# wei-zeng98/piano-a2s

Measured on AMD Instinct MI355X. Metric: training clips/sec (12 s, 5-bar), higher is better.
Workload: dtype f32

## Files before the change

### include/a2s.h

```cpp
#ifndef A2S_H
#define A2S_H
#include <stddef.h>
#include <stdint.h>
#ifdef __cplusplus
extern "C" {
#endif

#define A2S_OK 0
#define A2S_ERR_ARG (-1)
#define A2S_ERR_HIP (-2)
#define A2S_ERR_WORKSPACE (-3)

const char* a2s_last_error(void);
int a2s_version(void);
long long a2s_launch_count(void);

int a2s_gemm_f32(void* stream, int M, int N, int K, float alpha, const float* A, long sAm, long sAk,
                 const float* B, long sBk, long sBn, float beta, float* C, long ldc, const float* bias, int act,
                 int batch, long bsA, long bsB, long bsC, int splitk, float* workspace, size_t workspace_bytes);
int a2s_gemm_f32_affine(void* stream, int M, int N, int K, float alpha, const float* A, long sAm, long sAk, const float* B, long sBk,
                        long sBn, float beta, float* C, long ldc, const float* bias, int act, int batch, long bsA, long bsB, long bsC,
                        int splitk, float* workspace, size_t workspace_bytes, const float* a_scale, const float* a_shift, int a_period,
                        const float* b_scale, const float* b_shift, int b_period);
int a2s_gemm_f32_bnstats(void* stream, int M, int N, int K, const float* A, long sAm, long sAk, const float* B, long sBk, long sBn, float* C, long ldc,
                         const float* y, const float* mean, const float* invstd, const float* scale, const float* shift, int period, float* partial);
int a2s_gemm_f32_affine_scaled(void* stream, int M, int N, int K, float alpha, const float* A, long sAm, long sAk, const float* B, long sBk,
                               long sBn, float beta, float* C, long ldc, const float* bias, int act, int batch, long bsA, long bsB, long bsC,
                               int splitk, float* workspace, size_t workspace_bytes, const float* a_scale, const float* a_shift, int a_period,
                               const float* b_scale, const float* b_shift, int b_period, const float* a_absmax, const float* b_absmax);
int a2s_gemm_f32_bnstats_scaled(void* stream, int M, int N, int K, const float* A, long sAm, long sAk, const float* B, long sBk, long sBn, float* C, long ldc,
                                const float* y, const float* mean, const float* invstd, const float* scale, const float* shift, int period, float* partial,
                                const float* a_absmax, const float* b_absmax);
int a2s_linear_dgrad_bnstats(void* stream, int M, int N, int K, const float* dz, long lda, const float* Wt, float* da, long ldc, const float* y,
                             const float* mean, const float* invstd, const float* scale, const float* shift, int period, float* partial,
                             const float* dz_absmax, const float* w_absmax, float* workspace, size_t workspace_bytes, float* da_absmax_out);
int a2s_linear_fwd(void* stream, int M, int N, int K, const float* y, long lda, const float* W, float* z, long ldc, const float* scale, const float* shift,
                   int period, const float* y_absmax, const float* w_absmax, float* workspace, size_t workspace_bytes);
int a2s_linear_fwd_eligible(int M, int N, int K, int period);
int a2s_linear_wgrad(void* stream, int M, int N, int K, const float* dz, long ldz, const float* y, long lda, float* G, long ldg, const float* scale,
                     const float* shift, int period, const float* dz_absmax, const float* y_absmax, float* workspace, size_t workspace_bytes);
size_t a2s_linear_wgrad_ws_bytes(int M, int K);
int a2s_linear_wgrad_eligible(int M, int N, int K, int period);
int a2s_tallk_wgrad(void* stream, int M, int Np, int K, const float* P, long ldp, const float* A, long lda, float* G, long ldg, int transposed, float* bias,
                    const float* p_absmax, const float* a_absmax, float* workspace, size_t workspace_bytes);
size_t a2s_tallk_wgrad_ws_bytes(int M, int Np, int K);
int a2s_tallk_wgrad_eligible(int M, int Np, int K, long ldp, long lda, long ldg, int transposed);
size_t a2s_linear_dgrad_ws_bytes(int N, int K);
int a2s_linear_dgrad_blocks(int M);
int a2s_linear_dgrad_eligible(int M, int N, int K, int period);
int a2s_absmax(void* stream, const float* x, long n, float* out);
int a2s_gemm_bnstats_blocks(int M, int period);
size_t a2s_gemm_workspace_bytes(int M, int N, int batch, int splitk);
int a2s_gemm_pick_splitk(int M, int N, int K, int batch);
void a2s_gemm_debug_tile(int cfg);
int a2s_debug_set(const char* key, int value);
int a2s_debug_get(const char* key);
int a2s_env_check(void);
int a2s_persist_abort_latch(void* device_word);

int a2s_conv3x3(void* stream, const float* x, const float* w, float* y, const float* in_scale, const float* in_shift,
                float* stat_partial, int B, int T, int F, int Cin, int Cout, int flip, float* workspace);
int a2s_conv3x3_ranged(void* stream, const float* x, const float* w, float* y, const float* in_scale, const float* in_shift, const float* in_absmax,
                       float* stat_partial, float* out_absmax, int B, int T, int F, int Cin, int Cout, float* workspace);
int a2s_conv3x3_stat_blocks(int B, int T, int F, int Cin);
int a2s_conv3x3_dgrad_bnstats(void* stream, const float* dy, const float* w, float* g, const float* yl, const float* yl_mean, const float* yl_invstd,
                              const float* yl_scale, const float* yl_shift, float* stat_partial, int B, int T, int F, int Cin, int Cout,
                              float* workspace);
int a2s_bn_bwd_from_partial(void* stream, const float* g, const float* x, const float* mean, const float* invstd, const float* scale, const float* shift,
                            float* dgamma, float* dbeta, float* dx , const float* partial, int nblocks, float* c12, long rows, int C, int F);
int a2s_conv3x3_dgrad_bnstats_scaled(void* stream, const float* dy, const float* w, float* g, const float* yl, const float* yl_mean, const float* yl_invstd,
                                     const float* yl_scale, const float* yl_shift, float* stat_partial, int B, int T, int F, int Cin, int Cout,
                                     float* workspace, const float* dy_absmax);
int a2s_conv3x3_dgrad_bnstats_ranged(void* stream, const float* dy, const float* w, float* g, const float* yl, const float* yl_mean, const float* yl_invstd,
                                     const float* yl_scale, const float* yl_shift, float* stat_partial, int B, int T, int F, int Cin, int Cout,
                                     float* workspace, const float* dy_absmax, float* g_absmax_out);
int a2s_bn_bwd_from_partial_amax(void* stream, const float* g, const float* x, const float* mean, const float* invstd, const float* scale, const float* shift,
                                 float* dgamma, float* dbeta, float* dx, const float* partial, int nblocks, float* c12, long rows, int C, int F,
                                 float* dx_absmax);
size_t a2s_conv3x3_workspace_floats(int Cin);
int a2s_bn_finalize(void* stream, const float* partial, int nblocks, int C, double count, const float* gamma,
                    const float* beta, float* running_mean, float* running_var, long long* num_batches_tracked,
                    float* mean, float* invstd, float* scale, float* shift, float eps, float momentum, int training);
int a2s_bn_relu_apply(void* stream, const float* x, float* y, const float* scale, const float* shift, long n, int C, int F);
int a2s_col_stats(void* stream, const float* x, float* partial, long rows, int C, int rows_per_block);
int a2s_bn1d_relu_dropout(void* stream, const float* x, float* y, const float* scale, const float* shift,
                          const uint8_t* keep_mask, float inv_keep, long n, int C);

int a2s_gru_gates_fwd(void* stream, const float* gi, long ldgi, const float* gh, long ldgh, const float* hprev, long ldhp,
                      float* hout, long ldho, float* hout2, long ldho2, float* save, int R, int H);
int a2s_gru_seq_fwd(void* stream, const float* gi_all, long gi_bstride, long gi_tstride, const float* w_hh,
                    const float* b_hh, float* out, long out_bstride, long out_tstride, float* hbuf, float* gh,
                    float* save, float* hn, int B, int T, int H, int reverse, float* workspace, size_t workspace_bytes);

int a2s_attn_step_fwd(void* stream, const float* keys, const float* enc, const float* q, long ldq, const float* v,
                      float* ctx, long ldctx, float* ctx2, long ldctx2, float* attw, int B, int T, int H,
                      const int* n_done, int n_rows_total, float* workspace);
int a2s_attn_step_fwd_rows(void* stream, const float* keys, const float* enc, const float* q, long ldq, const float* v, float* ctx,
                           long ldctx, float* ctx2, long ldctx2, float* attw, int R, int T, int H, float* workspace, int n_clips,
                           const int* clip_order, const int* clip_rank, const int* row_until, int n_active, int step);
size_t a2s_attn_workspace_floats(int B, int T, int H);
size_t a2s_attn_workspace_floats_fused(int n_clips, int T, int H, int groups);

int a2s_log_softmax_rows(void* stream, const float* x, long ldx, float* y, long ldy, int* argmax_out, int R, int V);
int a2s_embed_rows(void* stream, const float* table, const long long* ids64, const int* ids32, long id_stride,
                   int const_id, float* out, long ldo, int col0, int R, int E, const uint8_t* keep_mask, float inv_keep);

typedef struct a2s_note_dec_args {
    const float* attn_w; const float* attn_b; const float* attn_v;
    const float* w_ih; const float* w_hh; const float* b_ih; const float* b_hh;
    const float* out_w; const float* out_b; const float* emb;
    const float* keys; const float* enc;
    float* h; float* x; float* q; float* gates; float* attw; float* o;
    float* gh; float* gi; float* logits;
    float* probs; long probs_bstride;
    const long long* gt; long gt_bstride;
    const uint8_t* tf_flags;
    const uint8_t* drop; float inv_keep;
    int* argmax_out; long am_bstride;
    int* eos_seen; long long* lengths; int* n_done;
    int* steps_exec;
    float* attn_ws;
    float* gemm_ws; size_t gemm_ws_bytes;
    int* t_base;
    const int* clip_order;
    const int* clip_rank;
    const int* row_until;
    const int* n_active;
    int n_clips;
    const int* m_active;
    const int* row_list;
    const int* n_rows_active;
    int R, T, H, E, V, steps, poll, eos_id;
    int use_graph;
    float* step_ws; size_t step_ws_floats;
    const int* tf_flags_dev;
// ... 201 lines not shown
```

### piano_a2s_amd/csrc/a2s_api.hip

```cpp
#define A2S_SWITCHES_IMPL
#include "a2s_internal.h"

thread_local char a2s_err_msg[512] = {0};
long long a2s_launch_counter = 0;

#define ST ((hipStream_t)stream)

extern "C" {

const char* a2s_last_error(void) { return a2s_err_msg; }
int a2s_version(void) { return 1; }
long long a2s_launch_count(void) { return __atomic_load_n(&a2s_launch_counter, __ATOMIC_RELAXED); }

int a2s_gemm_f32(void* stream, int M, int N, int K, float alpha, const float* A, long sAm, long sAk, const float* B, long sBk,
                 long sBn, float beta, float* C, long ldc, const float* bias, int act, int batch, long bsA, long bsB, long bsC,
                 int splitk, float* workspace, size_t workspace_bytes) {
    return a2s_gemm_impl(ST, M, N, K, alpha, A, sAm, sAk, B, sBk, sBn, beta, C, ldc, bias, act, batch, bsA, bsB, bsC, splitk,
                         workspace, workspace_bytes);
}
int a2s_gemm_f32_affine(void* stream, int M, int N, int K, float alpha, const float* A, long sAm, long sAk, const float* B, long sBk,
                        long sBn, float beta, float* C, long ldc, const float* bias, int act, int batch, long bsA, long bsB, long bsC,
                        int splitk, float* workspace, size_t workspace_bytes, const float* a_scale, const float* a_shift, int a_period,
                        const float* b_scale, const float* b_shift, int b_period) {
    return a2s_gemm_affine_impl(ST, M, N, K, alpha, A, sAm, sAk, B, sBk, sBn, beta, C, ldc, bias, act, batch, bsA, bsB, bsC, splitk,
                                workspace, workspace_bytes, a_scale, a_shift, a_period, b_scale, b_shift, b_period,
                                nullptr, nullptr, nullptr, nullptr, nullptr, nullptr, 0, 0, nullptr, nullptr);
}
int a2s_gemm_f32_affine_scaled(void* stream, int M, int N, int K, float alpha, const float* A, long sAm, long sAk, const float* B, long sBk,
                               long sBn, float beta, float* C, long ldc, const float* bias, int act, int batch, long bsA, long bsB, long bsC,
                               int splitk, float* workspace, size_t workspace_bytes, const float* a_scale, const float* a_shift, int a_period,
                               const float* b_scale, const float* b_shift, int b_period, const float* a_absmax, const float* b_absmax) {
    return a2s_gemm_affine_impl(ST, M, N, K, alpha, A, sAm, sAk, B, sBk, sBn, beta, C, ldc, bias, act, batch, bsA, bsB, bsC, splitk,
                                workspace, workspace_bytes, a_scale, a_shift, a_period, b_scale, b_shift, b_period,
                                nullptr, nullptr, nullptr, nullptr, nullptr, nullptr, 0, 1, a_absmax, b_absmax);
}
int a2s_gemm_f32_bnstats_scaled(void* stream, int M, int N, int K, const float* A, long sAm, long sAk, const float* B, long sBk, long sBn, float* C, long ldc,
                                const float* y, const float* mean, const float* invstd, const float* scale, const float* shift, int period, float* partial,
                                const float* a_absmax, const float* b_absmax) {
    return a2s_gemm_affine_impl(ST, M, N, K, 1.f, A, sAm, sAk, B, sBk, sBn, 0.f, C, ldc, nullptr, 0, 1, 0, 0, 0, 1, nullptr, 0,
                                nullptr, nullptr, 0, nullptr, nullptr, 0, y, mean, invstd, scale, shift, partial, period, 1, a_absmax, b_absmax);
}
int a2s_absmax(void* stream, const float* x, long n, float* out) { return a2s_absmax_impl(ST, x, n, out); }
int a2s_linear_dgrad_bnstats(void* stream, int M, int N, int K, const float* dz, long lda, const float* Wt, float* da, long ldc, const float* y,
                             const float* mean, const float* invstd, const float* scale, const float* shift, int period, float* partial,
                             const float* dz_absmax, const float* w_absmax, float* workspace, size_t workspace_bytes, float* da_absmax_out) {
    return a2s_linear_dgrad_bnstats_impl(ST, M, N, K, dz, lda, Wt, 1, K, da, ldc, y, mean, invstd, scale, shift, period, partial, dz_absmax, w_absmax,
                                         workspace, workspace_bytes, da_absmax_out);
}
size_t a2s_linear_dgrad_ws_bytes(int N, int K) { return a2s_linear_dgrad_ws_bytes_impl(N, K); }
int a2s_linear_fwd(void* stream, int M, int N, int K, const float* y, long lda, const float* W, float* z, long ldc, const float* scale, const float* shift,
                   int period, const float* y_absmax, const float* w_absmax, float* workspace, size_t workspace_bytes) {
    return a2s_linear_fwd_impl(ST, M, N, K, y, lda, W, z, ldc, scale, shift, period, y_absmax, w_absmax, workspace, workspace_bytes);
}
int a2s_linear_wgrad(void* stream, int M, int N, int K, const float* dz, long ldz, const float* y, long lda, float* G, long ldg, const float* scale,
                     const float* shift, int period, const float* dz_absmax, const float* y_absmax, float* workspace, size_t workspace_bytes) {
    return a2s_linear_wgrad_impl(ST, M, N, K, dz, ldz, y, lda, G, ldg, scale, shift, period, dz_absmax, y_absmax, workspace, workspace_bytes);
}
size_t a2s_linear_wgrad_ws_bytes(int M, int K) { return a2s_linear_wgrad_ws_bytes_impl(M, K); }
int a2s_linear_wgrad_eligible(int M, int N, int K, int period) { return a2s_linear_wgrad_ok(M, N, K, 256, 4, 4, period, nullptr, nullptr, nullptr) ? 1 : 0; }
int a2s_tallk_wgrad(void* stream, int M, int Np, int K, const float* P, long ldp, const float* A, long lda, float* G, long ldg, int transposed, float* bias,
                    const float* p_absmax, const float* a_absmax, float* workspace, size_t workspace_bytes) {
    return a2s_tallk_wgrad_impl(ST, M, Np, K, P, ldp, A, lda, G, ldg, transposed, bias, p_absmax, a_absmax, workspace, workspace_bytes);
}
size_t a2s_tallk_wgrad_ws_bytes(int M, int Np, int K) { return a2s_tallk_wgrad_ws_bytes_impl(M, Np, K); }
int a2s_tallk_wgrad_eligible(int M, int Np, int K, long ldp, long lda, long ldg, int transposed) {
    return a2s_tallk_wgrad_ok(M, Np, K, ldp, lda, ldg, transposed, nullptr, nullptr, nullptr, nullptr) ? 1 : 0;
}
int a2s_linear_fwd_eligible(int M, int N, int K, int period) { return a2s_linear_fwd_ok(M, N, K, 4, 4, period, nullptr, nullptr, nullptr) ? 1 : 0; }
int a2s_linear_dgrad_blocks(int M) { return a2s_linear_dgrad_blocks_impl(M); }
int a2s_linear_dgrad_eligible(int M, int N, int K, int period) {
    return a2s_linear_dgrad_ok(M, N, K, 4, 1, K, 4, period, nullptr, nullptr, nullptr, nullptr) ? 1 : 0;
}
int a2s_gemm_f32_bnstats(void* stream, int M, int N, int K, const float* A, long sAm, long sAk, const float* B, long sBk, long sBn, float* C, long ldc,
                         const float* y, const float* mean, const float* invstd, const float* scale, const float* shift, int period, float* partial) {
    return a2s_gemm_affine_impl(ST, M, N, K, 1.f, A, sAm, sAk, B, sBk, sBn, 0.f, C, ldc, nullptr, 0, 1, 0, 0, 0, 1, nullptr, 0,
                                nullptr, nullptr, 0, nullptr, nullptr, 0, y, mean, invstd, scale, shift, partial, period, 0, nullptr, nullptr);
}
int a2s_gemm_bnstats_blocks(int M, int period) { return a2s_cdiv(M, 128) * a2s_gemm_bnstats_slots(period); }
size_t a2s_gemm_workspace_bytes(int M, int N, int batch, int splitk) { return a2s_gemm_workspace_bytes_impl(M, N, batch, splitk); }
int a2s_gemm_pick_splitk(int M, int N, int K, int batch) { return a2s_gemm_pick_splitk_impl(M, N, K, batch); }
void a2s_gemm_debug_tile(int cfg) { a2s_gemm_debug_tile_impl(cfg); }
size_t a2s_note_step_workspace_floats(int H, int E) { return a2s_note_step_workspace_floats_impl(H, E); }
int a2s_debug_set(const char* key, int value) {
    if (!key) return A2S_ERR_ARG;
    const int id = a2s_switch_find(key);
    if (id >= 0) { a2s_switch_store(id, value); return A2S_OK; }
    if (!strcmp(key, "attn_deferred_fast")) { a2s_attn_deferred_fast = value ? 1 : 0; return A2S_OK; }
    if (!strcmp(key, "tallk_wgrad")) { a2s_tallk_wgrad_on = value ? 1 : 0; return A2S_OK; }
    if (!strcmp(key, "tallk_wgrad_max_splits")) { a2s_tallk_wgrad_max_splits = value > 0 ? value : 0; return A2S_OK; }
    if (!strcmp(key, "gemm_tile")) { a2s_gemm_debug_tile_impl(value); return A2S_OK; }
    snprintf(a2s_err_msg, sizeof(a2s_err_msg), "a2s_debug_set: unknown key %s", key);
    return A2S_ERR_ARG;
}
int a2s_env_check(void) {
    if (const char* e = a2s_switch_env_error()) A2S_FAIL(A2S_ERR_ARG, "%s: expected a decimal number >= 0", e);
    return A2S_OK;
}

int a2s_persist_abort_latch(void* device_word) { a2s_persist_latch_set(device_word); return A2S_OK; }

int a2s_debug_get(const char* key) {
    if (!key) return -1;
    const int id = a2s_switch_find(key);
    if (id == A2S_SW_attn_pair_fused_rows) return a2s_attn_pair_fused_rows();
    if (id >= 0) return a2s_sw((a2s_switch)id);
    if (!strcmp(key, "attn_pair_launches")) return (int)a2s_attn_pair_launches();
    if (!strcmp(key, "attn_pair_bwd_launches")) return (int)a2s_attn_pair_bwd_launches();
    if (!strcmp(key, "attn_deferred_fast")) return a2s_attn_deferred_fast;
    if (!strcmp(key, "tallk_wgrad")) return a2s_tallk_wgrad_on;
    if (!strcmp(key, "tallk_wgrad_max_splits")) return a2s_tallk_wgrad_max_splits;
    if (!strcmp(key, "tallk_wgrad_launches")) return (int)a2s_tallk_wgrad_launches();
    if (!strcmp(key, "attn_dk_ahead_launches")) return (int)a2s_attn_dk_ahead_launches();
    if (!strcmp(key, "attn_denc_launches")) return (int)a2s_attn_denc_launches();
    if (!strcmp(key, "dec_mid_launches")) return a2s_dec_mid_launches();
    if (!strcmp(key, "dec_persist_launches")) return a2s_dec_persist_launches();
    if (!strcmp(key, "edit_distance_launches")) return (int)a2s_edit_distance_launches();
    if (!strcmp(key, "conv_rows16_c20_launches")) return (int)a2s_conv_rows16_c20_launches();
    if (!strcmp(key, "device_cus")) return a2s_device_geometry().cus;
    if (!strcmp(key, "device_xccs")) return a2s_device_geometry().xccs;
    return -1;
}

int a2s_conv3x3(void* stream, const float* x, const float* w, float* y, const float* in_scale, const float* in_shift,
                float* stat_partial, int B, int T, int F, int Cin, int Cout, int flip, float* workspace) {
    return a2s_conv3x3_impl(ST, x, w, y, in_scale, in_shift, stat_partial, B, T, F, Cin, Cout, flip, workspace, nullptr, nullptr, nullptr, nullptr, nullptr, nullptr,
                            nullptr, nullptr);
}
int a2s_conv3x3_ranged(void* stream, const float* x, const float* w, float* y, const float* in_scale, const float* in_shift, const float* in_absmax,
                       float* stat_partial, float* out_absmax, int B, int T, int F, int Cin, int Cout, float* workspace) {
    return a2s_conv3x3_impl(ST, x, w, y, in_scale, in_shift, stat_partial, B, T, F, Cin, Cout, 0, workspace, nullptr, nullptr, nullptr, nullptr, nullptr, nullptr,
                            in_absmax, out_absmax);
}
int a2s_conv3x3_dgrad_bnstats(void* stream, const float* dy, const float* w, float* g, const float* yl, const float* yl_mean, const float* yl_invstd,
                              const float* yl_scale, const float* yl_shift, float* stat_partial, int B, int T, int F, int Cin, int Cout,
                              float* workspace) {
    if (!yl) { snprintf(a2s_err_msg, sizeof(a2s_err_msg), "conv3x3_dgrad_bnstats: yl is required"); return A2S_ERR_ARG; }
    return a2s_conv3x3_impl(ST, dy, w, g, nullptr, nullptr, stat_partial, B, T, F, Cin, Cout, 1, workspace, yl, yl_mean, yl_invstd, yl_scale, yl_shift, nullptr, nullptr, nullptr);
}
int a2s_conv3x3_dgrad_bnstats_scaled(void* stream, const float* dy, const float* w, float* g, const float* yl, const float* yl_mean, const float* yl_invstd,
                                     const float* yl_scale, const float* yl_shift, float* stat_partial, int B, int T, int F, int Cin, int Cout,
                                     float* workspace, const float* dy_absmax) {
    if (!yl) { snprintf(a2s_err_msg, sizeof(a2s_err_msg), "conv3x3_dgrad_bnstats_scaled: yl is required"); return A2S_ERR_ARG; }
    return a2s_conv3x3_impl(ST, dy, w, g, nullptr, nullptr, stat_partial, B, T, F, Cin, Cout, 1, workspace, yl, yl_mean, yl_invstd, yl_scale, yl_shift, dy_absmax, nullptr, nullptr);
}
int a2s_conv3x3_dgrad_bnstats_ranged(void* stream, const float* dy, const float* w, float* g, const float* yl, const float* yl_mean, const float* yl_invstd,
                                     const float* yl_scale, const float* yl_shift, float* stat_partial, int B, int T, int F, int Cin, int Cout,
                                     float* workspace, const float* dy_absmax, float* g_absmax_out) {
    if (!yl) { snprintf(a2s_err_msg, sizeof(a2s_err_msg), "conv3x3_dgrad_bnstats_ranged: yl is required"); return A2S_ERR_ARG; }
    return a2s_conv3x3_impl(ST, dy, w, g, nullptr, nullptr, stat_partial, B, T, F, Cin, Cout, 1, workspace, yl, yl_mean, yl_invstd, yl_scale, yl_shift, dy_absmax, nullptr, g_absmax_out);
}
int a2s_bn_bwd_from_partial(void* stream, const float* g, const float* x, const float* mean, const float* invstd, const float* scale, const float* shift,
                            float* dgamma, float* dbeta, float* dx, const float* partial, int nblocks, float* c12, long rows, int C, int F) {
    return a2s_bn_bwd_from_partial_impl(ST, g, x, mean, invstd, scale, shift, dgamma, dbeta, dx, partial, nblocks, c12, rows, C, F, nullptr);
}
int a2s_bn_bwd_from_partial_amax(void* stream, const float* g, const float* x, const float* mean, const float* invstd, const float* scale, const float* shift,
                                 float* dgamma, float* dbeta, float* dx, const float* partial, int nblocks, float* c12, long rows, int C, int F,
                                 float* dx_absmax) {
    return a2s_bn_bwd_from_partial_impl(ST, g, x, mean, invstd, scale, shift, dgamma, dbeta, dx, partial, nblocks, c12, rows, C, F, dx_absmax);
}
size_t a2s_conv3x3_workspace_floats(int Cin) { return a2s_conv3x3_workspace_floats_impl(Cin); }
int a2s_conv3x3_stat_blocks(int B, int T, int F, int Cin) { return a2s_conv3x3_stat_blocks_impl(B, T, F, Cin); }
int a2s_bn_finalize(void* stream, const float* partial, int nblocks, int C, double count, const float* gamma, const float* beta,
                    float* running_mean, float* running_var, long long* nbt, float* mean, float* invstd, float* scale,
                    float* shift, float eps, float momentum, int training) {
    return a2s_bn_finalize_impl(ST, partial, nblocks, C, count, gamma, beta, running_mean, running_var, nbt, mean, invstd, scale,
                                shift, eps, momentum, training);
}
int a2s_bn_relu_apply(void* stream, const float* x, float* y, const float* scale, const float* shift, long n, int C, int F) {
    return a2s_bn_relu_apply_impl(ST, x, y, scale, shift, n, C, F);
}
int a2s_col_stats(void* stream, const float* x, float* partial, long rows, int C, int rows_per_block) {
    return a2s_col_stats_impl(ST, x, partial, rows, C, rows_per_block);
}
int a2s_bn1d_relu_dropout(void* stream, const float* x, float* y, const float* scale, const float* shift, const uint8_t* keep_mask,
                          float inv_keep, long n, int C) {
    return a2s_bn1d_relu_dropout_impl(ST, x, y, scale, shift, keep_mask, inv_keep, n, C);
}
int a2s_gru_gates_fwd(void* stream, const float* gi, long ldgi, const float* gh, long ldgh, const float* hprev, long ldhp,
                      float* hout, long ldho, float* hout2, long ldho2, float* save, int R, int H) {
    return a2s_gru_gates_fwd_impl(ST, gi, ldgi, gh, ldgh, hprev, ldhp, hout, ldho, hout2, ldho2, save, R, H);
}
int a2s_gru_seq_fwd(void* stream, const float* gi_all, long gi_bstride, long gi_tstride, const float* w_hh, const float* b_hh,
                    float* out, long out_bstride, long out_tstride, float* hbuf, float* gh, float* save, float* hn, int B, int T,
                    int H, int reverse, float* workspace, size_t workspace_bytes) {
    return a2s_gru_seq_fwd_impl(ST, gi_all, gi_bstride, gi_tstride, w_hh, b_hh, out, out_bstride, out_tstride, hbuf, gh, save, hn,
                                B, T, H, reverse, workspace, workspace_bytes);
}
int a2s_attn_step_fwd(void* stream, const float* keys, const float* enc, const float* q, long ldq, const float* v, float* ctx,
                      long ldctx, float* ctx2, long ldctx2, float* attw, int B, int T, int H, const int* n_done, int n_rows_total, float* workspace) {
    return a2s_attn_step_fwd_impl(ST, keys, enc, q, ldq, v, ctx, ldctx, ctx2, ldctx2, attw, B, T, H, n_done, n_rows_total, workspace, nullptr);
}
int a2s_attn_step_fwd_rows(void* stream, const float* keys, const float* enc, const float* q, long ldq, const float* v, float* ctx,
// ... 285 lines not shown
```

### piano_a2s_amd/csrc/a2s_common.h

```cpp
#pragma once
#include <hip/hip_runtime.h>
#include <stdint.h>
#include <stdio.h>
#include <string.h>

#define A2S_OK 0
#define A2S_ERR_ARG (-1)
#define A2S_ERR_HIP (-2)
#define A2S_ERR_WORKSPACE (-3)

extern thread_local char a2s_err_msg[512];

#define A2S_FAIL(code, ...)                                   \
    do {                                                      \
        snprintf(a2s_err_msg, sizeof(a2s_err_msg), __VA_ARGS__); \
        return (code);                                        \
    } while (0)

#define A2S_REQUIRE(cond, ...)                 \
    do {                                       \
        if (!(cond)) A2S_FAIL(A2S_ERR_ARG, __VA_ARGS__); \
    } while (0)

#define A2S_CHECK_LAUNCH(name)                                                        \
// ... 64 lines not shown
}
#define A2S_DPP_QUAD_1032 0xB1
#define A2S_DPP_QUAD_2301 0x4E
#define A2S_DPP_ROW_HALF_MIRROR 0x141
#define A2S_DPP_ROW_MIRROR 0x140
#define A2S_DPP_ROW_BCAST15 0x142
#define A2S_DPP_ROW_BCAST31 0x143
__device__ __forceinline__ float wave_sum_lane63(float v) {
    v += dpp_take<A2S_DPP_QUAD_1032>(0.f, v);
    v += dpp_take<A2S_DPP_QUAD_2301>(0.f, v);
    v += dpp_take<A2S_DPP_ROW_HALF_MIRROR>(0.f, v);
    v += dpp_take<A2S_DPP_ROW_MIRROR>(0.f, v);
    v += dpp_take<A2S_DPP_ROW_BCAST15, 0xA>(0.f, v);
    v += dpp_take<A2S_DPP_ROW_BCAST31, 0xC>(0.f, v);
    return v;
}
__device__ __forceinline__ float wave_sum(float v) {
    return __builtin_bit_cast(float, __builtin_amdgcn_readlane(__builtin_bit_cast(int, wave_sum_lane63(v)), 63));
}
__device__ __forceinline__ float wave_max(float v) {
    v = fmaxf(v, dpp_take<A2S_DPP_QUAD_1032>(v, v));
    v = fmaxf(v, dpp_take<A2S_DPP_QUAD_2301>(v, v));
    v = fmaxf(v, dpp_take<A2S_DPP_ROW_HALF_MIRROR>(v, v));
    v = fmaxf(v, dpp_take<A2S_DPP_ROW_MIRROR>(v, v));
    v = fmaxf(v, dpp_take<A2S_DPP_ROW_BCAST15, 0xA, false>(v, v));
    v = fmaxf(v, dpp_take<A2S_DPP_ROW_BCAST31, 0xC, false>(v, v));
    return __builtin_bit_cast(float, __builtin_amdgcn_readlane(__builtin_bit_cast(int, v), 63));
}
__device__ __forceinline__ float attn_merge_weight(float mg, float lg, bool have, float& m_out, float& inv_l_out) {
#pragma clang fp contract(off)
    const float m = wave_max(mg);
    const float d = mg - m;
    const float e = have ? __expf(d) : 0.f;
    const float t = lg * e;
    const float l = wave_sum(t);
    m_out = m;
    inv_l_out = 1.f / l;
    return e / l;
}
struct GruCellGrad { float dr, dz, dn, dnr, dhz; };
__device__ __forceinline__ GruCellGrad gru_cell_bwd(float dh, float rg, float zg, float ng, float ghn, float hp) {
#pragma clang fp contract(off)
    GruCellGrad o;
    o.dn = dh * (1.f - zg) * (1.f - ng * ng);
    o.dz = dh * (hp - ng) * zg * (1.f - zg);
    o.dr = o.dn * ghn * rg * (1.f - rg);
    o.dnr = o.dn * rg;
    o.dhz = dh * zg;
    return o;
}
__device__ __forceinline__ double wave_sum_d(double v) {
#pragma unroll
    for (int o = 32; o > 0; o >>= 1) v += __shfl_xor(v, o, 64);
    return v;
}

__device__ __forceinline__ float block_sum(float v, float* red) {
    v = wave_sum(v);
    const int w = threadIdx.x >> 6, nw = (blockDim.x + 63) >> 6;
    __syncthreads();
    if ((threadIdx.x & 63) == 0) red[w] = v;
    __syncthreads();
    float t = 0.f;
    for (int i = 0; i < nw; ++i) t += red[i];
    return t;
}
__device__ __forceinline__ float block_max(float v, float* red) {
    v = wave_max(v);
    const int w = threadIdx.x >> 6, nw = (blockDim.x + 63) >> 6;
    __syncthreads();
    if ((threadIdx.x & 63) == 0) red[w] = v;
    __syncthreads();
    float t = red[0];
    for (int i = 1; i < nw; ++i) t = fmaxf(t, red[i]);
    return t;
}

__device__ __forceinline__ float fast_tanh(float x) {
    x = fminf(fmaxf(x, -15.f), 15.f);
    const float e = __expf(2.f * x);
    return fmaf(-2.f, __builtin_amdgcn_rcpf(e + 1.f), 1.f);
}
__device__ __forceinline__ float exp2x_clamped(float x) { return __expf(2.f * fminf(fmaxf(x, -43.f), 43.f)); }
__device__ __forceinline__ float tanh_ek(float ek, float eq) { return fmaf(-2.f, __builtin_amdgcn_rcpf(fmaf(ek, eq, 1.f)), 1.f); }
__device__ __forceinline__ float sech2_ek(float ek, float eq) {
    const float r = __builtin_amdgcn_rcpf(fmaf(ek, eq, 1.f));
    return 4.f * r * (1.f - r);
}
__device__ __forceinline__ float fast_sigmoid(float x) {
    x = fminf(fmaxf(x, -30.f), 30.f);
    return __builtin_amdgcn_rcpf(1.f + __expf(-x));
}
typedef __attribute__((ext_vector_type(8))) __bf16 bf16x8;
typedef __attribute__((ext_vector_type(2))) __bf16 bf16x2;
typedef __attribute__((ext_vector_type(2))) float f32x2;
__device__ __forceinline__ void split3_pair(float x0, float x1, unsigned& p0, unsigned& p1, unsigned& p2) {
    f32x2 v = {x0, x1};
    p0 = __builtin_bit_cast(unsigned, __builtin_convertvector(v, bf16x2));
    v[0] -= __uint_as_float(p0 << 16); v[1] -= __uint_as_float(p0 & 0xffff0000u);
    p1 = __builtin_bit_cast(unsigned, __builtin_convertvector(v, bf16x2));
    v[0] -= __uint_as_float(p1 << 16); v[1] -= __uint_as_float(p1 & 0xffff0000u);
    p2 = __builtin_bit_cast(unsigned, __builtin_convertvector(v, bf16x2));
}

typedef __attribute__((ext_vector_type(8))) _Float16 f16x8;
typedef __attribute__((ext_vector_type(2))) _Float16 f16x2;
__device__ __forceinline__ void split2_pair_f16(float x0, float x1, unsigned& p0, unsigned& p1) {
    f32x2 v = {x0, x1};
    const f16x2 t0 = __builtin_convertvector(v, f16x2);
    p0 = __builtin_bit_cast(unsigned, t0);
    asm("v_fma_mix_f32 %0, %1, -1.0, %0 op_sel_hi:[1,0,0]" : "+v"(v[0]) : "v"(p0));
    asm("v_fma_mix_f32 %0, %1, -1.0, %0 op_sel:[1,0,0] op_sel_hi:[1,0,0]" : "+v"(v[1]) : "v"(p0));
    p1 = __builtin_bit_cast(unsigned, __builtin_convertvector(v, f16x2));
}
__device__ __forceinline__ void block_absmax_to(float* __restrict__ out, float am, float* red) {
    am = block_max(am, red);
    if (threadIdx.x == 0) {
        const unsigned bits = __float_as_uint(am);
        if (bits > __hip_atomic_load(reinterpret_cast<unsigned*>(out), __ATOMIC_RELAXED, __HIP_MEMORY_SCOPE_AGENT))
            atomicMax(reinterpret_cast<unsigned*>(out), bits);
    }
}
__device__ __forceinline__ int pow2_scale_exp(float amax, int target) {
    if (!(amax > 0.f) || !isfinite(amax)) return 0;
    const int k = target - ilogbf(amax);
    return min(max(k, -96), 96);
}

#endif
```

### piano_a2s_amd/csrc/a2s_gemm.hip

```cpp
#include "a2s_internal.h"

struct GemmArgs {
    const float* A; const float* B; float* C; const float* bias;
    int M, N, K;
    long sAm, sAk, sBk, sBn, ldc;
    float alpha, beta;
    int act;
    int batch; long bsA, bsB, bsC;
    int splitk; int kchunk;
    float* partial;
    int vecA, vecB;
    const float* a_scale; const float* a_shift; int a_period;
    const float* b_scale; const float* b_shift; int b_period;
    const float* ep_y; const float* ep_mean; const float* ep_invstd; const float* ep_scale; const float* ep_shift;
    float* ep_partial; int ep_period, ep_channels, ep_slots;
    int two_term; const float* a_absmax; const float* b_absmax;
};

#define GEMM_BK 32
#ifndef GEMM_DEPTH
#define GEMM_DEPTH 1
#endif

template <int ROWS, bool KC> struct LdsTile {
// ... 309 lines not shown
#pragma unroll
            for (int i = 0; i < TM; ++i)
#pragma unroll
                for (int j = 0; j < TN; ++j)
#pragma unroll
                    for (int r = 0; r < 4; ++r) acc[i][j][r] *= unscale;
        }
    } else {
        constexpr int D = (BM * BN <= 64 * 64) ? GEMM_DEPTH : 1;
        f32x4 qa[D][NLA], qb[D][NLB];
        float ga[D][NLA][2], gb[D][NLB][2];
#pragma unroll
        for (int i = 0; i < NLA; ++i) { qa[0][i] = ra[i]; ga[0][i][0] = fa[i][0]; ga[0][i][1] = fa[i][1]; }
#pragma unroll
        for (int i = 0; i < NLB; ++i) { qb[0][i] = rb[i]; gb[0][i][0] = fb[i][0]; gb[0][i][1] = fb[i][1]; }
#pragma unroll
        for (int d = 1; d < D; ++d) {
            if (d < ntiles) {
                const int k0 = kbeg + d * GEMM_BK;
                tile_load<BM, A_KC, NLA>(A, g.sAm, g.sAk, m0, k0, g.M, kend, g.vecA, qa[d], ga[d], g.a_scale, g.a_shift, g.a_period);
                tile_load<BN, B_KC, NLB>(B, g.sBn, g.sBk, n0, k0, g.N, kend, g.vecB, qb[d], gb[d], g.b_scale, g.b_shift, g.b_period);
            }
        }
        for (int t0 = 0; t0 < ntiles; t0 += D) {
#pragma unroll
            for (int d = 0; d < D; ++d) {
                const int t = t0 + d;
                if (t >= ntiles) break;
                float* la = lds + (t & 1) * (LA::SIZE + LB::SIZE);
                float* lb = la + LA::SIZE;
                tile_store<BM, A_KC, NLA>(la, qa[d], ga[d], m0, kbeg + t * GEMM_BK, g.M, kend, g.a_scale, g.a_shift, g.a_period);
                tile_store<BN, B_KC, NLB>(lb, qb[d], gb[d], n0, kbeg + t * GEMM_BK, g.N, kend, g.b_scale, g.b_shift, g.b_period);
                __syncthreads();
                if (t + D < ntiles) {
                    const int k0 = kbeg + (t + D) * GEMM_BK;
                    tile_load<BM, A_KC, NLA>(A, g.sAm, g.sAk, m0, k0, g.M, kend, g.vecA, qa[d], ga[d], g.a_scale, g.a_shift, g.a_period);
                    tile_load<BN, B_KC, NLB>(B, g.sBn, g.sBk, n0, k0, g.N, kend, g.vecB, qb[d], gb[d], g.b_scale, g.b_shift, g.b_period);
                }
#pragma unroll
                for (int ks = 0; ks < GEMM_BK / 4; ++ks) {
                    float a[TM], b[TN];
#pragma unroll
                    for (int i = 0; i < TM; ++i) a[i] = la[LA::at(wm + i * 16 + lr, ks * 4 + lk)];
#pragma unroll
                    for (int j = 0; j < TN; ++j) b[j] = lb[LB::at(wn + j * 16 + lr, ks * 4 + lk)];
#pragma unroll
                    for (int i = 0; i < TM; ++i)
#pragma unroll
                        for (int j = 0; j < TN; ++j)
                            acc[i][j] = __builtin_amdgcn_mfma_f32_16x16x4f32(b[j], a[i], acc[i][j], 0, 0, 0);
                }
            }
        }
    }


    const bool partial = g.splitk > 1;
    float* C = partial ? g.partial + (long)blockIdx.z * g.M * g.N : g.C + (long)zb * g.bsC;
    const long ldc = partial ? g.N : g.ldc;
    const bool vec_c = (ldc % 4 == 0) && (((uintptr_t)C & 15) == 0);
    const int ep_c0 = g.ep_y ? n0 / g.ep_period : 0;
    float ep_s[2][2] = {{0.f, 0.f}, {0.f, 0.f}};
#pragma unroll
    for (int i = 0; i < TM; ++i) {
        const int m = m0 + wm + i * 16 + lr;
        if (m >= g.M) continue;
#pragma unroll
        for (int j = 0; j < TN; ++j) {
            const int n = n0 + wn + j * 16 + lk * 4;
            if (n >= g.N) continue;
            f32x4 v = acc[i][j];
            float* dst = C + (long)m * ldc + n;
            const bool full = vec_c && n + 3 < g.N;
            if (!partial) {
                f32x4 old = {0.f, 0.f, 0.f, 0.f};
                if (g.beta != 0.f) {
                    if (full) old = *reinterpret_cast<const f32x4*>(dst);
                    else {
#pragma unroll
                        for (int r = 0; r < 4; ++r) if (n + r < g.N) old[r] = dst[r];
                    }
                }
#pragma unroll
                for (int r = 0; r < 4; ++r) {
                    float x = g.alpha * v[r] + ((g.bias && n + r < g.N) ? g.bias[n + r] : 0.f);
                    if (g.beta != 0.f) x += g.beta * old[r];
                    if (g.act == 1) x = fmaxf(x, 0.f);
                    else if (g.act == 2) x = fast_tanh(x);
                    else if (g.act == 3) x = exp2x_clamped(x);
                    v[r] = x;
                }
            }
            if (full) *reinterpret_cast<f32x4*>(dst) = v;
            else {
#pragma unroll
                for (int r = 0; r < 4; ++r) if (n + r < g.N) dst[r] = v[r];
            }
            if (g.ep_y && full) {
                const int c = n / g.ep_period;
                const f32x4 yq = *reinterpret_cast<const f32x4*>(g.ep_y + (long)m * ldc + n);
                const float mean = g.ep_mean[c], invstd = g.ep_invstd[c], sc = g.ep_scale[c], sh = g.ep_shift[c];
                float a1 = 0.f, a2 = 0.f;
#pragma unroll
                for (int r = 0; r < 4; ++r) {
                    const float gm = (yq[r] * sc + sh > 0.f) ? v[r] : 0.f;
                    a1 += gm; a2 += gm * (yq[r] - mean) * invstd;
                }
                if (c == ep_c0) { ep_s[0][0] += a1; ep_s[0][1] += a2; } else { ep_s[1][0] += a1; ep_s[1][1] += a2; }
            }
        }
    }
    if (g.ep_y) {
        float* red = lds;
        __syncthreads();
#pragma unroll
        for (int sl = 0; sl < 2; ++sl)
#pragma unroll
            for (int k = 0; k < 2; ++k) {
                const float w = wave_sum(ep_s[sl][k]);
                if (lane == 0) red[wave * 4 + sl * 2 + k] = w;
            }
        __syncthreads();
        if (threadIdx.x < 4) {
            const int sl = threadIdx.x >> 1, k = threadIdx.x & 1;
            const int c = ep_c0 + sl;
            if (c < g.ep_channels && (long)c * g.ep_period < (long)n0 + BN) {
                float tot = 0.f;
#pragma unroll
                for (int w = 0; w < WM * WN; ++w) tot += red[w * 4 + threadIdx.x];
                const int slot = bx - (int)(((long)c * g.ep_period) / BN);
                g.ep_partial[(((long)by * g.ep_slots + slot) * g.ep_channels + c) * 2 + k] = tot;
            }
        }
    }
}

__global__ void gemm_splitk_reduce(GemmArgs g) {
    const long mn = (long)g.M * g.N;
    const long idx = (long)blockIdx.x * blockDim.x + threadIdx.x;
    const int zb = blockIdx.y;
    if (idx >= mn) return;
    const float* p = g.partial + (long)zb * g.splitk * mn + idx;
    float s = 0.f;
    for (int i = 0; i < g.splitk; ++i) s += p[(long)i * mn];
    const int m = (int)(idx / g.N), n = (int)(idx % g.N);
    float* c = g.C + (long)zb * g.bsC + (long)m * g.ldc + n;
    float v = g.alpha * s + (g.bias ? g.bias[n] : 0.f);
    if (g.beta != 0.f) v += g.beta * *c;
    if (g.act == 1) v = fmaxf(v, 0.f);
    else if (g.act == 2) v = fast_tanh(v);
    else if (g.act == 3) v = exp2x_clamped(v);
    *c = v;
}

__global__ __launch_bounds__(256) void absmax_kernel(const float* __restrict__ x, long n, float* __restrict__ out) {
    float m = 0.f;
    for (long i = (long)blockIdx.x * 256 + threadIdx.x; i < n; i += (long)gridDim.x * 256) m = fmaxf(m, fabsf(x[i]));
    __shared__ float red[16];
    block_absmax_to(out, m, red);
}
int a2s_absmax_impl(hipStream_t st, const float* x, long n, float* out) {
    A2S_REQUIRE(x && out && n >= 0, "absmax: null tensor");
    hipError_t e = hipMemsetAsync(out, 0, sizeof(float), st);
    if (e != hipSuccess) A2S_FAIL(A2S_ERR_HIP, "absmax memset: %s", hipGetErrorString(e));
    if (n == 0) return A2S_OK;
    hipLaunchKernelGGL(absmax_kernel, dim3((unsigned)min((long)1024, (n + 255) / 256)), dim3(256), 0, st, x, n, out);
    A2S_CHECK_LAUNCH("absmax_kernel");
    return A2S_OK;
}

template <int BM, int BN, int WM, int WN>
static void launch_cfg(const GemmArgs& g, bool akc, bool bkc, hipStream_t st) {
    dim3 grid(a2s_cdiv(g.N, BN), a2s_cdiv(g.M, BM), g.batch * g.splitk);
    if constexpr (BM == 128 && BN == 128) {
        const bool a_ok = akc || (g.sAm == 1 && g.vecA), b_ok = bkc || (g.sBn == 1 && g.vecB);
        if (a2s_sw(A2S_SW_gemm_bf16x3) && g.K >= (g.two_term ? 128 : 256) && a_ok && b_ok) {
            if (g.two_term && a2s_sw(A2S_SW_gemm_f16x2)) {
                if (akc && bkc) hipLaunchKernelGGL((gemm_f32_kernel<BM, BN, WM, WN, true, true, 2>), grid, dim3(256), 0, st, g);
                else if (akc) hipLaunchKernelGGL((gemm_f32_kernel<BM, BN, WM, WN, true, false, 2>), grid, dim3(256), 0, st, g);
                else if (bkc) hipLaunchKernelGGL((gemm_f32_kernel<BM, BN, WM, WN, false, true, 2>), grid, dim3(256), 0, st, g);
                else hipLaunchKernelGGL((gemm_f32_kernel<BM, BN, WM, WN, false, false, 2>), grid, dim3(256), 0, st, g);
                return;
            }
            if (akc && bkc) hipLaunchKernelGGL((gemm_f32_kernel<BM, BN, WM, WN, true, true, 3>), grid, dim3(256), 0, st, g);
            else if (akc) hipLaunchKernelGGL((gemm_f32_kernel<BM, BN, WM, WN, true, false, 3>), grid, dim3(256), 0, st, g);
            else if (bkc) hipLaunchKernelGGL((gemm_f32_kernel<BM, BN, WM, WN, false, true, 3>), grid, dim3(256), 0, st, g);
            else hipLaunchKernelGGL((gemm_f32_kernel<BM, BN, WM, WN, false, false, 3>), grid, dim3(256), 0, st, g);
            return;
        }
    }
    const size_t pad = (BM * BN <= 64 * 64 && g.M >= 256 && a2s_sw(A2S_SW_attn_bulk_cap)) ? 16384 : 0;
    if (akc && bkc) hipLaunchKernelGGL((gemm_f32_kernel<BM, BN, WM, WN, true, true>), grid, dim3(256), pad, st, g);
    else if (akc && !bkc) hipLaunchKernelGGL((gemm_f32_kernel<BM, BN, WM, WN, true, false>), grid, dim3(256), pad, st, g);
    else if (!akc && bkc) hipLaunchKernelGGL((gemm_f32_kernel<BM, BN, WM, WN, false, true>), grid, dim3(256), pad, st, g);
    else hipLaunchKernelGGL((gemm_f32_kernel<BM, BN, WM, WN, false, false>), grid, dim3(256), pad, st, g);
}

static bool big_two_term_ok(const GemmArgs& g, bool akc, bool bkc) {
    const bool a_ok = akc || (g.sAm == 1 && g.vecA), b_ok = bkc || (g.sBn == 1 && g.vecB);
    return g.two_term && a2s_sw(A2S_SW_gemm_f16x2) && a2s_sw(A2S_SW_gemm_bf16x3) && (!g.ep_y || g.ep_period >= 256) && g.K >= 128 && a_ok && b_ok && g.M >= 256 && g.N >= 256 &&
           (long)a2s_cdiv(g.M, 256) * a2s_cdiv(g.N, 256) * g.batch * g.splitk >= 192;
}
static void launch_big_two_term(const GemmArgs& g, bool akc, bool bkc, hipStream_t st) {
    dim3 grid(a2s_cdiv(g.N, 256), a2s_cdiv(g.M, 256), g.batch * g.splitk);
    if (akc && bkc) hipLaunchKernelGGL((gemm_f32_kernel<256, 256, 4, 2, true, true, 2>), grid, dim3(512), 0, st, g);
    else if (akc) hipLaunchKernelGGL((gemm_f32_kernel<256, 256, 4, 2, true, false, 2>), grid, dim3(512), 0, st, g);
    else if (bkc) hipLaunchKernelGGL((gemm_f32_kernel<256, 256, 4, 2, false, true, 2>), grid, dim3(512), 0, st, g);
    else hipLaunchKernelGGL((gemm_f32_kernel<256, 256, 4, 2, false, false, 2>), grid, dim3(512), 0, st, g);
}

size_t a2s_gemm_workspace_bytes_impl(int M, int N, int batch, int splitk) {
    return splitk > 1 ? (size_t)batch * splitk * M * N * sizeof(float) : 0;
}

int a2s_gemm_pick_splitk_impl(int M, int N, int K, int batch) {
    const long tiles = (long)a2s_cdiv(M, 64) * a2s_cdiv(N, 64) * batch;
    if (K < 4096) return 1;
    if (tiles >= 256) {
        const long t128 = (long)a2s_cdiv(M, 128) * a2s_cdiv(N, 128) * batch;
        if (t128 >= 2048 || K < 32768) return 1;
        const long t256 = (long)a2s_cdiv(M, 256) * a2s_cdiv(N, 256) * batch;
        int best = 1; double best_eff = 0.0;
        for (int s = 1; s <= 12; ++s) {
            const long wg = t128 * s, wg2 = t256 * s;
            double eff = (double)wg / (double)(a2s_cdiv(wg, 512) * 512);
            if (M >= 256 && N >= 256) eff = fmin(eff, (double)wg2 / (double)(a2s_cdiv(wg2, 256) * 256));
            if (eff > best_eff + 0.02) { best_eff = eff; best = s; }
        }
        return best;
    }
    const long t128 = (long)a2s_cdiv(M, 128) * a2s_cdiv(N, 128) * batch;
    if (K >= 8192 && t128 >= 12) {
        long s = a2s_cdiv(256, t128);
        if (s > K / 2048) s = K / 2048;
        if (s > 16) s = 16;
        if (s >= 1 && t128 * s >= 192) return (int)s;
    }
    long s = 512 / tiles;
    const long maxs = K / 512;
    if (s > maxs) s = maxs;
    if (s > 64) s = 64;
    return s < 1 ? 1 : (int)s;
}

int a2s_gemm_bnstats_slots(int period) { return period > 0 ? (period + 127) / 128 + 1 : 0; }

static int g_force_tile = 0;
void a2s_gemm_debug_tile_impl(int cfg) { g_force_tile = cfg; }

int a2s_gemm_affine_impl(hipStream_t st, int M, int N, int K, float alpha, const float* A, long sAm, long sAk,
                  const float* B, long sBk, long sBn, float beta, float* C, long ldc, const float* bias, int act,
                  int batch, long bsA, long bsB, long bsC, int splitk, float* ws, size_t ws_bytes,
                  const float* a_scale, const float* a_shift, int a_period, const float* b_scale, const float* b_shift, int b_period,
                  const float* ep_y, const float* ep_mean, const float* ep_invstd, const float* ep_scale, const float* ep_shift,
                  float* ep_partial, int ep_period, int two_term, const float* a_absmax, const float* b_absmax) {
    if (M <= 0 || N <= 0 || batch <= 0) return A2S_OK;
    A2S_REQUIRE(K >= 0 && A && B && C, "gemm: null operand or negative K");
    A2S_REQUIRE(splitk >= 0, "gemm: splitk must be >= 0 (0 = choose automatically when a workspace is given)");
    const bool mid = M > 64 && M <= 2048 && batch == 1 && N <= 2048;
    int mid_tile = 0;
    if (mid) mid_tile = M <= 1024 ? 2 : 3;
    if (splitk == 0) {
        splitk = 1;
        if (mid) {
            const long tiles = (long)a2s_cdiv(M, 64) * a2s_cdiv(N, mid_tile == 2 ? 32 : 64);
            if (ws && tiles < 256 && K >= 512 && a2s_gemm_workspace_bytes_impl(M, N, batch, 4) <= ws_bytes) splitk = 4;
        } else {
            const long bm = M <= 16 ? 16 : (M <= 32 ? 32 : 64), bn = M <= 64 ? (M <= 16 ? 64 : (M <= 32 ? 64 : 32)) : 64;
            const long tiles = (long)a2s_cdiv(M, bm) * a2s_cdiv(N, bn) * batch;
            if (ws && tiles < 192 && K >= 256) {
                long s = (256 + tiles - 1) / tiles;
                if (s > K / 64) s = K / 64;
                if (s > 16) s = 16;
                while (s > 1 && a2s_gemm_workspace_bytes_impl(M, N, batch, (int)s) > ws_bytes) --s;
                if (s > 1) splitk = (int)s;
            }
        }
    } else {
        mid_tile = 0;
    }
    GemmArgs g;
    g.A = A; g.B = B; g.C = C; g.bias = bias; g.M = M; g.N = N; g.K = K;
    g.sAm = sAm; g.sAk = sAk; g.sBk = sBk; g.sBn = sBn; g.ldc = ldc; g.alpha = alpha; g.beta = beta; g.act = act;
    g.batch = batch; g.bsA = bsA; g.bsB = bsB; g.bsC = bsC;
    g.splitk = splitk; g.partial = ws;
    g.two_term = two_term; g.a_absmax = a_absmax; g.b_absmax = b_absmax;
    A2S_REQUIRE((a_scale == nullptr) == (a_shift == nullptr) && (b_scale == nullptr) == (b_shift == nullptr), "gemm: operand scale/shift must come together");
    A2S_REQUIRE((!a_scale || a_period > 0) && (!b_scale || b_period > 0), "gemm: operand affine needs a positive period");
    A2S_REQUIRE(!a_scale || sAk == 1 || sAm == 1, "gemm: operand affine needs a unit-stride dimension on A");
    A2S_REQUIRE(!b_scale || sBk == 1 || sBn == 1, "gemm: operand affine needs a unit-stride dimension on B");
    g.a_scale = a_scale; g.a_shift = a_shift; g.a_period = a_period > 0 ? a_period : 1;
    g.b_scale = b_scale; g.b_shift = b_shift; g.b_period = b_period > 0 ? b_period : 1;
    g.ep_y = ep_y; g.ep_mean = ep_mean; g.ep_invstd = ep_invstd; g.ep_scale = ep_scale; g.ep_shift = ep_shift; g.ep_partial = ep_partial;
    g.ep_period = ep_period > 0 ? ep_period : 1; g.ep_channels = ep_y ? N / g.ep_period : 0; g.ep_slots = ep_y ? a2s_gemm_bnstats_slots(ep_period) : 0;
    if (ep_y) {
        A2S_REQUIRE(ep_mean && ep_invstd && ep_scale && ep_shift && ep_partial && ep_period >= 128 && ep_period % 4 == 0 && N % ep_period == 0,
                    "gemm: the BatchNorm-statistics epilogue needs its tensors, period >= 128, period %% 4 == 0, N a multiple of the period");
        A2S_REQUIRE(splitk == 1 && batch == 1 && M > 64 && ldc % 4 == 0 && ((uintptr_t)C % 16 == 0) && ((uintptr_t)ep_y % 16 == 0) && beta == 0.f,
                    "gemm: the BatchNorm-statistics epilogue needs one split, one batch, M > 64, beta 0 and 16-byte aligned rows");
        hipError_t e = hipMemsetAsync(ep_partial, 0, sizeof(float) * 2 * (size_t)a2s_cdiv(M, 128) * g.ep_slots * g.ep_channels, st);
        if (e != hipSuccess) A2S_FAIL(A2S_ERR_HIP, "gemm bn-stats memset: %s", hipGetErrorString(e));
    }
    g.kchunk = a2s_cdiv(a2s_cdiv(K, splitk), GEMM_BK) * GEMM_BK;
    if (g.kchunk == 0) g.kchunk = GEMM_BK;
    if (splitk > 1)
        A2S_REQUIRE(ws && ws_bytes >= a2s_gemm_workspace_bytes_impl(M, N, batch, splitk), "gemm: split-K workspace too small");
    const bool akc = (sAk == 1) || (sAm != 1);
    const bool bkc = (sBk == 1) || (sBn != 1);
    auto aligned = [](const void* p, long s0, long s1) { return ((uintptr_t)p % 16 == 0) && (s0 % 4 == 0) && (s1 % 4 == 0); };
    g.vecA = (akc ? (sAk == 1 && aligned(A, sAm, bsA)) : (sAm == 1 && aligned(A, sAk, bsA))) ? 1 : 0;
    g.vecB = (bkc ? (sBk == 1 && aligned(B, sBn, bsB)) : (sBn == 1 && aligned(B, sBk, bsB))) ? 1 : 0;

    if (!g_force_tile && big_two_term_ok(g, akc, bkc)) launch_big_two_term(g, akc, bkc, st);
    else if (ep_y) launch_cfg<128, 128, 2, 2>(g, akc, bkc, st);
    else if (!g_force_tile && mid_tile == 2 && g.splitk >= 1 && M * (long)N < (1L << 22)) launch_cfg<64, 32, 4, 1>(g, akc, bkc, st);
    else if (!g_force_tile && mid_tile == 3 && M * (long)N < (1L << 22)) launch_cfg<64, 64, 2, 2>(g, akc, bkc, st);
    else if (g_force_tile && M > 64) {
        switch (g_force_tile) {
            case 1: launch_cfg<32, 64, 2, 2>(g, akc, bkc, st); break;
            case 2: launch_cfg<64, 32, 4, 1>(g, akc, bkc, st); break;
            case 3: launch_cfg<64, 64, 2, 2>(g, akc, bkc, st); break;
            default: launch_cfg<128, 128, 2, 2>(g, akc, bkc, st); break;
        }
    }
    else if (M <= 16) launch_cfg<16, 64, 1, 4>(g, akc, bkc, st);
    else if (M <= 32) launch_cfg<32, 64, 2, 2>(g, akc, bkc, st);
    else if (M <= 64) launch_cfg<64, 32, 4, 1>(g, akc, bkc, st);
    else if ((long)a2s_cdiv(M, 128) * a2s_cdiv(N, 128) * batch * splitk >= 192) launch_cfg<128, 128, 2, 2>(g, akc, bkc, st);
    else launch_cfg<64, 64, 2, 2>(g, akc, bkc, st);
    A2S_CHECK_LAUNCH("gemm_f32_kernel");
    if (splitk > 1) {
        dim3 grid(a2s_cdiv((long)M * N, 256), batch);
        hipLaunchKernelGGL(gemm_splitk_reduce, grid, dim3(256), 0, st, g);
        A2S_CHECK_LAUNCH("gemm_splitk_reduce");
    }
    return A2S_OK;
}

int a2s_gemm_impl(hipStream_t st, int M, int N, int K, float alpha, const float* A, long sAm, long sAk,
                  const float* B, long sBk, long sBn, float beta, float* C, long ldc, const float* bias, int act,
                  int batch, long bsA, long bsB, long bsC, int splitk, float* ws, size_t ws_bytes) {
    return a2s_gemm_affine_impl(st, M, N, K, alpha, A, sAm, sAk, B, sBk, sBn, beta, C, ldc, bias, act, batch, bsA, bsB, bsC, splitk, ws, ws_bytes,
                                nullptr, nullptr, 0, nullptr, nullptr, 0, nullptr, nullptr, nullptr, nullptr, nullptr, nullptr, 0, 0, nullptr, nullptr);
}
```

### piano_a2s_amd/csrc/a2s_internal.h

```cpp
#pragma once
#include "a2s_common.h"
#include "../../include/a2s.h"
#include "a2s_switches.h"

static inline int a2s_attn_pair_fused_rows(void) {
    const int cap = a2s_sw(A2S_SW_dec_fused_max_rows), v = a2s_sw(A2S_SW_attn_pair_fused_rows);
    return v < cap ? v : cap;
}
static inline unsigned a2s_persist_dbg(void) {
    return (a2s_sw(A2S_SW_persist_force_agent) ? PERSIST_DBG_FORCE_AGENT : 0u) | (a2s_sw(A2S_SW_persist_inject_abort) ? PERSIST_DBG_INJECT_ABORT : 0u);
}

int a2s_absmax_impl(hipStream_t st, const float* x, long n, float* out);
size_t a2s_gemm_workspace_bytes_impl(int M, int N, int batch, int splitk);
int a2s_gemm_pick_splitk_impl(int M, int N, int K, int batch);
int a2s_gemm_bnstats_slots(int period);
void a2s_gemm_debug_tile_impl(int cfg);
int a2s_gemm_affine_impl(hipStream_t st, int M, int N, int K, float alpha, const float* A, long sAm, long sAk,
    const float* B, long sBk, long sBn, float beta, float* C, long ldc, const float* bias, int act,
    int batch, long bsA, long bsB, long bsC, int splitk, float* ws, size_t ws_bytes,
    const float* a_scale, const float* a_shift, int a_period, const float* b_scale, const float* b_shift, int b_period,
    const float* ep_y, const float* ep_mean, const float* ep_invstd, const float* ep_scale, const float* ep_shift,
    float* ep_partial, int ep_period, int two_term, const float* a_absmax, const float* b_absmax);
int a2s_gemm_impl(hipStream_t st, int M, int N, int K, float alpha, const float* A, long sAm, long sAk,
    const float* B, long sBk, long sBn, float beta, float* C, long ldc, const float* bias, int act,
    int batch, long bsA, long bsB, long bsC, int splitk, float* ws, size_t ws_bytes);

size_t a2s_linear_dgrad_ws_bytes_impl(int N, int K);
int a2s_linear_dgrad_blocks_impl(int M);
bool a2s_linear_dgrad_ok(int M, int N, int K, long lda, long sBk, long sBn, long ldc, int period, const void* A, const void* B, const void* C, const void* y);
int a2s_linear_dgrad_bnstats_impl(hipStream_t st, int M, int N, int K, const float* A, long lda, const float* Wt, long sBk, long sBn, float* C, long ldc,
    const float* ep_y, const float* mean, const float* invstd, const float* scale, const float* shift, int period,
    float* partial, const float* a_absmax, const float* b_absmax, float* ws, size_t ws_bytes, float* c_absmax_out);
bool a2s_linear_fwd_ok(int M, int N, int K, long lda, long ldc, int period, const void* A, const void* W, const void* C);
int a2s_linear_fwd_impl(hipStream_t st, int M, int N, int K, const float* A, long lda, const float* W, float* C, long ldc, const float* a_scale,
    const float* a_shift, int period, const float* a_absmax, const float* w_absmax, float* ws, size_t ws_bytes);
size_t a2s_linear_wgrad_ws_bytes_impl(int M, int K);
bool a2s_linear_wgrad_ok(int M, int N, int K, long ldz, long lda, long ldg, int period, const void* dz, const void* A, const void* G);
int a2s_linear_wgrad_impl(hipStream_t st, int M, int N, int K, const float* dz, long ldz, const float* A, long lda, float* G, long ldg, const float* a_scale,
    const float* a_shift, int period, const float* dz_absmax, const float* a_absmax, float* ws, size_t ws_bytes);
extern int a2s_tallk_wgrad_on;
extern int a2s_tallk_wgrad_max_splits;
long a2s_tallk_wgrad_launches(void);
size_t a2s_tallk_wgrad_ws_bytes_impl(int M, int Np, int K);
bool a2s_tallk_wgrad_ok(int M, int Np, int K, long ldp, long lda, long ldg, int transposed, const void* P, const void* A, const void* G, const void* bias);
int a2s_tallk_wgrad_impl(hipStream_t st, int M, int Np, int K, const float* P, long ldp, const float* A, long lda, float* G, long ldg, int transposed,
    float* bias, const float* p_absmax, const float* a_absmax, float* ws, size_t ws_bytes);

int a2s_act_bound_impl(hipStream_t st, const float* scale, const float* shift, const float* absmax, int C, float* out);
size_t a2s_conv3x3_workspace_floats_impl(int Cin);
int a2s_conv3x3_impl(hipStream_t st, const float* x, const float* w, float* y, const float* in_scale,
    const float* in_shift, float* stat_partial, int B, int T, int F, int Cin, int Cout, int flip, float* ws,
    const float* yl, const float* yl_mean, const float* yl_invstd, const float* yl_scale, const float* yl_shift,
    const float* x_absmax, const float* in_absmax, float* out_absmax);
int a2s_conv3x3_stat_blocks_impl(int B, int T, int F, int Cin);
int a2s_bn_finalize_impl(hipStream_t st, const float* partial, int nblocks, int C, double count, const float* gamma,
    const float* beta, float* running_mean, float* running_var, long long* nbt, float* mean,
    float* invstd, float* scale, float* shift, float eps, float momentum, int training);
int a2s_bn_relu_apply_impl(hipStream_t st, const float* x, float* y, const float* scale, const float* shift, long n, int C, int F);
int a2s_col_stats_impl(hipStream_t st, const float* x, float* partial, long rows, int C, int rows_per_block);
int a2s_bn1d_relu_dropout_impl(hipStream_t st, const float* x, float* y, const float* scale, const float* shift,
    const uint8_t* mask, float inv_keep, long n, int C);
size_t a2s_conv3x3_wgrad_workspace_bytes_impl(int Cin, int Cout);
int a2s_conv3x3_wgrad_impl(hipStream_t st, const float* dy, const float* x, const float* in_scale, const float* in_shift, float* dW,
    float* ws, size_t ws_bytes, int B, int T, int F, int Cin, int Cout, const float* bn_y, const float* bn_mean,
    const float* bn_invstd, const float* bn_scale, const float* bn_shift, const float* bn_c12, float* dy_out,
    const float* dy_absmax, const float* act_absmax);
int a2s_bn_bwd_impl(hipStream_t st, const float* g, const float* x, const float* mean, const float* invstd, const float* scale,
    const float* shift, const uint8_t* mask, float inv_keep, float* dgamma, float* dbeta, float* dx, float* partial,
    float* c12, long rows, int C, int F, float* dx_absmax);
int a2s_bn_bwd_from_partial_impl(hipStream_t st, const float* g, const float* x, const float* mean, const float* invstd, const float* scale,
    const float* shift, float* dgamma, float* dbeta, float* dx, const float* partial, int nblocks, float* c12,
    long rows, int C, int F, float* dx_absmax);
int a2s_bn_bwd_stats_impl(hipStream_t st, const float* g, const float* x, const float* mean, const float* invstd, const float* scale,
    const float* shift, const uint8_t* mask, float inv_keep, float* partial, float* sums, long rows, int C, int F);
int a2s_bn_bwd_apply_impl(hipStream_t st, const float* g, const float* x, const float* mean, const float* invstd, const float* scale,
    const float* shift, const uint8_t* mask, float inv_keep, const float* sums_local, const float* sums_global,
    double count_global, float* dgamma, float* dbeta, float* dx, float* c12, long rows, int C, int F);
int a2s_bn_bwd_sums_from_partial_impl(hipStream_t st, const float* partial, int nblocks, int C, float* sums);
int a2s_bn_bwd_c12_from_sums_impl(hipStream_t st, const float* sums_local, const float* sums_global, double count_global, float* dgamma, float* dbeta,
    float* c12, int C);
size_t a2s_bn_bwd_partial_floats_impl(long rows, int C, int F);

int a2s_channel_absmax_impl(hipStream_t st, const float* x, long rows, int C, int F, float* out);
bool a2s_conv_rows_eligible(int F, int Cin);
int a2s_conv_rows_blocks(int B, int T, int F);
size_t a2s_conv_rows_workspace_floats(int Cin);
long a2s_conv_rows16_c20_launches(void);
int a2s_conv3x3_rows_impl(hipStream_t st, const float* x, const float* w, float* y, const float* in_scale, const float* in_shift,
    const float* in_absmax, float* stat_partial, float* out_absmax, int B, int T, int F, int Cin, int Cout, int flip,
    float* ws, const float* yl, const float* yl_mean, const float* yl_invstd, const float* yl_scale, const float* yl_shift,
    const float* x_absmax);

bool a2s_wgrad_rows_eligible(int F, int Cin, int Cout);
int a2s_conv3x3_wgrad_rows_bn_impl(hipStream_t st, const float* g, const float* y, const float* mean, const float* invstd, const float* scale,
    const float* shift, const float* c12, const float* g_absmax, int g_absmax_n, const float* y_absmax, float* dz_out,
    float* dz_absmax_out, const float* x, const float* in_scale, const float* in_shift, float* dW, float* ws, size_t ws_bytes,
    int B, int T, int F, int Cin, int Cout, const float* act_absmax);
int a2s_conv3x3_wgrad_rows_impl(hipStream_t st, const float* dy, const float* x, const float* in_scale, const float* in_shift, float* dW, float* ws,
    size_t ws_bytes, int B, int T, int F, int Cin, int Cout, const float* dy_absmax, const float* act_absmax);

struct StepFinArgs {
    const float* logits; long ldl;
    float* probs; long probs_bstride;
    const long long* gt; long gt_bstride;
    const float* emb;
    float* xnext; long ldx;
    const uint8_t* drop; float inv_keep;
    int* argmax_out; long am_bstride;
    int* eos_seen; long long* lengths; int* n_done; int* steps_exec;
    const int* t_base;
    const int* row_until;
    int n_clips;
    int R, V, E, t, teacher_force, eos_id, max_t;
};
struct a2s_grammar_ref { const signed char* next; int n_states; int* row_state; };
int a2s_gru_gates_fwd_impl(hipStream_t st, const float* gi, long ldgi, const float* gh, long ldgh, const float* hprev,
    long ldhp, float* hout, long ldho, float* hout2, long ldho2, float* save, int R, int H);
int a2s_gru_bptt_step_impl(hipStream_t st, const float* dgh, const float* w_hh_t, const float* dhz_in, const float* dout, long ld_dout,
    const float* save, const float* hprev, long ld_hprev, float* dgi, long ld_dgi, float* dgh_out, float* dgh2,
    long ld_dgh2, float* dhz_out, int R, int H);
int a2s_skinny_gemm_acc_impl(hipStream_t st, const float* A, long lda, const float* Bt, long ldb, float* Cm, long ldc, int R, int N, int K);
int a2s_gru_seq_fwd_impl(hipStream_t st, const float* gi_all, long gi_bstride, long gi_tstride, const float* w_hh,
    const float* b_hh, float* out, long out_bstride, long out_tstride, float* hbuf, float* gh,
    float* save, float* hn, int B, int T, int H, int reverse, float* ws, size_t ws_bytes);
int a2s_attn_step_fwd_impl(hipStream_t st, const float* Kmat, const float* enc, const float* q, long ldq, const float* v,
    float* ctx, long ldctx, float* ctx2, long ldctx2, float* attw, int B, int T, int H,
    const int* n_done, int n_rows_total, float* ws, const a2s_attn_rows* rows = nullptr, a2s_attn_deferred* defer = nullptr);
int a2s_log_softmax_rows_impl(hipStream_t st, const float* x, long ldx, float* y, long ldy, int* argmax_out, int R, int V);
int a2s_embed_rows_impl(hipStream_t st, const float* table, const long long* ids64, const int* ids32, long id_stride,
// ... 219 lines not shown
```

### piano_a2s_amd/csrc/a2s_linear.hip

```cpp
#include "a2s_internal.h"

#define LIN_BM 128
#define LIN_K 256
#define LIN_RS 288
#define LIN_NTH 512
#define LIN_LDS (2 * 2 * LIN_BM * LIN_RS)

typedef unsigned lu32x4 __attribute__((ext_vector_type(4)));

struct LinDgradArgs {
    const float* A; long lda;
    const unsigned char* planes;
    float* C; long ldc;
    const float* ep_y;
    const float* mean; const float* invstd; const float* scale; const float* shift;
    float* partial;
    const float* a_absmax; const float* b_absmax;
    int M, N, period, channels;
    float* c_absmax_out;
};

__global__ __launch_bounds__(256) void lin_pack_planes_k(const float* __restrict__ W, long ld, int N, int K, const float* __restrict__ absmax,
                                                         unsigned char* __restrict__ out) {
    const long id = (long)blockIdx.x * 256 + threadIdx.x;
    const int kgroups = K >> 3, nks = K >> 5;
    const int n = (int)(id / kgroups), kg = (int)(id % kgroups);
    if (n >= N) return;
    const float ps = ldexpf(1.f, pow2_scale_exp(*absmax, 12));
    const f32x4 v0 = *reinterpret_cast<const f32x4*>(W + (long)n * ld + kg * 8);
    const f32x4 v1 = *reinterpret_cast<const f32x4*>(W + (long)n * ld + kg * 8 + 4);
    float x[8];
#pragma unroll
    for (int i = 0; i < 4; ++i) { x[i] = __builtin_amdgcn_fmed3f(v0[i] * ps, -65000.f, 65000.f); x[4 + i] = __builtin_amdgcn_fmed3f(v1[i] * ps, -65000.f, 65000.f); }
    lu32x4 hi, lo;
#pragma unroll
    for (int i = 0; i < 4; ++i) { unsigned h, l; split2_pair_f16(x[2 * i], x[2 * i + 1], h, l); hi[i] = h; lo[i] = l; }
    const int nt = n >> 4, lr = n & 15, ks = kg >> 2, lk = kg & 3;
    unsigned char* o = out + ((((long)nt * nks + ks) * 2) * 64 + (lk * 16 + lr)) * 16;
    *reinterpret_cast<lu32x4*>(o) = hi;
    *reinterpret_cast<lu32x4*>(o + 64 * 16) = lo;
}

__global__ __launch_bounds__(LIN_NTH) void lin_dgrad_bnstats(LinDgradArgs a) {
    __shared__ __attribute__((aligned(16))) unsigned char lds[LIN_LDS];
    const int tid = threadIdx.x, lane = tid & 63, wave = tid >> 6, lr = lane & 15, lk = lane >> 4;
    const int m0 = blockIdx.x * LIN_BM;
    const int ka = pow2_scale_exp(*a.a_absmax, 12), kb = pow2_scale_exp(*a.b_absmax, 12);
    const float psa = ldexpf(1.f, ka), unscale = ldexpf(1.f, -(ka + kb));

    {
        f32x4 v[16];
#pragma unroll
        for (int i = 0; i < 16; ++i) {
            const int slot = tid + LIN_NTH * i, row = slot >> 6, k = (slot & 63) * 4;
            v[i] = (f32x4){0.f, 0.f, 0.f, 0.f};
            if (m0 + row < a.M) v[i] = *reinterpret_cast<const f32x4*>(a.A + (long)(m0 + row) * a.lda + k);
        }
#pragma unroll
        for (int i = 0; i < 16; ++i) {
            const int slot = tid + LIN_NTH * i, row = slot >> 6, k = (slot & 63) * 4;
            float x[4];
#pragma unroll
            for (int j = 0; j < 4; ++j) x[j] = __builtin_amdgcn_fmed3f(v[i][j] * psa, -65000.f, 65000.f);
            uint2 hi, lo;
            split2_pair_f16(x[0], x[1], hi.x, lo.x);
            split2_pair_f16(x[2], x[3], hi.y, lo.y);
            const int blk = k >> 7, off = (k & 127) * 2;
            *reinterpret_cast<uint2*>(lds + ((blk * 2 + 0) * LIN_BM + row) * LIN_RS + off) = hi;
            *reinterpret_cast<uint2*>(lds + ((blk * 2 + 1) * LIN_BM + row) * LIN_RS + off) = lo;
        }
    }
    __syncthreads();

    const int ntiles = (a.N + 255) >> 8;
    const unsigned lane_off = (unsigned)(lr * a.ldc + lk * 4) * 4u;
    float s1 = 0.f, s2 = 0.f, vmax = 0.f;
    int cur_c = -1;
    auto flush = [&]() {
        if (cur_c < 0) return;
        const float w1 = wave_sum(s1), w2 = wave_sum(s2);
        if (lane == 0) {
            float* p = a.partial + (((long)blockIdx.x * 8 + wave) * a.channels + cur_c) * 2;
            p[0] = w1; p[1] = w2;
        }
    };
    lu32x4 bf[3][2][2];
    auto load_b = [&](int n0, int ks, lu32x4 (&dst)[2][2]) {
        const unsigned char* bp = a.planes + (long)(n0 >> 4) * 8 * 2 * 64 * 16;
#pragma unroll
        for (int nt = 0; nt < 2; ++nt)
#pragma unroll
            for (int sp = 0; sp < 2; ++sp) dst[nt][sp] = *reinterpret_cast<const lu32x4*>(bp + ((long)(nt * 8 + ks) * 2 + sp) * 1024 + (unsigned)lane * 16u);
    };
    if (wave * 32 < a.N) { load_b(wave * 32, 0, bf[0]); load_b(wave * 32, 1, bf[1]); }
    for (int j = 0; j < ntiles; ++j) {
        const int n0 = j * 256 + wave * 32;
        if (n0 >= a.N) break;
        f32x4 yq[8][2];
        auto load_y = [&](int mt) {
            const int m = m0 + mt * 16 + lr;
#pragma unroll
            for (int nt = 0; nt < 2; ++nt) {
#if defined(LIN_X) && LIN_X >= 1 && LIN_X != 4
                yq[mt][nt] = (f32x4){1.f, 1.f, 1.f, 1.f};
#else
                yq[mt][nt] = (f32x4){0.f, 0.f, 0.f, 0.f};
                if (m < a.M)
                    yq[mt][nt] = *reinterpret_cast<const f32x4*>(reinterpret_cast<const char*>(a.ep_y + (long)(m0 + mt * 16) * a.ldc + n0 + nt * 16) + lane_off);
#endif
            }
        };
// ... 21 lines not shown
                        af[sp][q] = *reinterpret_cast<const lu32x4*>(lds + (((ks >> 2) * 2 + sp) * LIN_BM + (half * 4 + q) * 16 + lr) * LIN_RS + (ks & 3) * 64 + lk * 16);
#define LIN_PRODUCT(SA, SB)                                                                                                   \
                _Pragma("unroll") for (int nt = 0; nt < 2; ++nt)                                                              \
                    _Pragma("unroll") for (int q = 0; q < 4; ++q)                                                             \
                        acc[half * 4 + q][nt] = __builtin_amdgcn_mfma_f32_16x16x32_f16(__builtin_bit_cast(f16x8, bf[ks % 3][nt][SB]), \
                                                                                       __builtin_bit_cast(f16x8, af[SA][q]), acc[half * 4 + q][nt], 0, 0, 0);
                LIN_PRODUCT(1, 0) LIN_PRODUCT(0, 1) LIN_PRODUCT(0, 0)
#undef LIN_PRODUCT
            }
        }
        if (n0 + 256 < a.N) { load_b(n0 + 256, 0, bf[0]); load_b(n0 + 256, 1, bf[1]); }
#pragma unroll
        for (int mt = 3; mt < 8; ++mt) load_y(mt);
        const int c = n0 / a.period;
        if (c != cur_c) { flush(); s1 = 0.f; s2 = 0.f; cur_c = c; }
        const float mean = a.mean[c], invstd = a.invstd[c], sc = a.scale[c], sh = a.shift[c];
#pragma unroll
        for (int mt = 0; mt < 8; ++mt) {
            const int m = m0 + mt * 16 + lr;
            if (m >= a.M) continue;
#pragma unroll
            for (int nt = 0; nt < 2; ++nt) {
                f32x4 v = acc[mt][nt];
#pragma unroll
                for (int r = 0; r < 4; ++r) { v[r] *= unscale; vmax = fmaxf(vmax, fabsf(v[r])); }
#if defined(LIN_X) && LIN_X >= 2
                if (v[0] == 123.456f)
#endif
                *reinterpret_cast<f32x4*>(reinterpret_cast<char*>(a.C + (long)(m0 + mt * 16) * a.ldc + n0 + nt * 16) + lane_off) = v;
#pragma unroll
                for (int r = 0; r < 4; ++r) {
                    const float gm = (fmaf(yq[mt][nt][r], sc, sh) > 0.f) ? v[r] : 0.f;
                    s1 += gm; s2 = fmaf(gm * (yq[mt][nt][r] - mean), invstd, s2);
                }
            }
        }
    }
    flush();
    if (a.c_absmax_out) {
        const float m = wave_max(vmax);
        if (lane == 0 && m > 0.f) atomicMax(reinterpret_cast<unsigned*>(a.c_absmax_out), __float_as_uint(m));
    }
}

size_t a2s_linear_dgrad_ws_bytes_impl(int N, int K) { return (K > 0 && K % 32 == 0 && N > 0) ? (size_t)N * K * 2 * 2 : 0; }
int a2s_linear_dgrad_blocks_impl(int M) { return M > 0 ? ((M + LIN_BM - 1) / LIN_BM) * 8 : 0; }

bool a2s_linear_dgrad_ok(int M, int N, int K, long lda, long sBk, long sBn, long ldc, int period, const void* A, const void* B, const void* C, const void* y) {
    return K == LIN_K && M >= LIN_BM && N >= 256 && N % 32 == 0 && period > 0 && period % 32 == 0 && N % period == 0 && N / period <= 4096 && sBk == 1 && sBn == K &&
           lda % 4 == 0 && ldc % 4 == 0 && (((uintptr_t)A | (uintptr_t)B | (uintptr_t)C | (uintptr_t)y) % 16 == 0);
}

int a2s_linear_dgrad_bnstats_impl(hipStream_t st, int M, int N, int K, const float* A, long lda, const float* Wt, long sBk, long sBn, float* C, long ldc,
                                  const float* ep_y, const float* mean, const float* invstd, const float* scale, const float* shift, int period,
                                  float* partial, const float* a_absmax, const float* b_absmax, float* ws, size_t ws_bytes, float* c_absmax_out) {
    A2S_REQUIRE(A && Wt && C && ep_y && mean && invstd && scale && shift && partial && a_absmax && b_absmax && ws, "linear_dgrad_bnstats: null argument");
    A2S_REQUIRE(a2s_linear_dgrad_ok(M, N, K, lda, sBk, sBn, ldc, period, A, Wt, C, ep_y),
                "linear_dgrad_bnstats: needs K = 256, M >= 128, N >= 256, N %% 32 == 0, period %% 32 == 0, a k-contiguous weight (N x K) and 16-byte aligned rows");
    A2S_REQUIRE(((uintptr_t)ws % 16 == 0) && ws_bytes >= a2s_linear_dgrad_ws_bytes_impl(N, K), "linear_dgrad_bnstats: workspace too small (%zu bytes needed)",
                a2s_linear_dgrad_ws_bytes_impl(N, K));
    const int channels = N / period, nblk = a2s_linear_dgrad_blocks_impl(M);
    hipError_t e = hipMemsetAsync(partial, 0, sizeof(float) * 2 * (size_t)nblk * channels, st);
    if (e != hipSuccess) A2S_FAIL(A2S_ERR_HIP, "linear_dgrad_bnstats memset: %s", hipGetErrorString(e));
    unsigned char* planes = reinterpret_cast<unsigned char*>(ws);
    hipLaunchKernelGGL(lin_pack_planes_k, dim3((unsigned)(((long)N * (K / 8) + 255) / 256)), dim3(256), 0, st, Wt, (long)K, N, K, b_absmax, planes);
    A2S_CHECK_LAUNCH("lin_pack_planes_k");
    LinDgradArgs a{A, lda, planes, C, ldc, ep_y, mean, invstd, scale, shift, partial, a_absmax, b_absmax, M, N, period, channels, c_absmax_out};
    hipLaunchKernelGGL(lin_dgrad_bnstats, dim3((M + LIN_BM - 1) / LIN_BM), dim3(LIN_NTH), 0, st, a);
    A2S_CHECK_LAUNCH("lin_dgrad_bnstats");
    return A2S_OK;
}

#define LF_RS 160
#define LF_STAGE (2 * LIN_BM * LF_RS)
#define LF_NS 3

struct LinFwdArgs {
    const float* A; long lda;
    const unsigned char* planes;
    float* C; long ldc;
    const float* a_scale; const float* a_shift;
    const float* a_absmax; const float* b_absmax;
    int M, K, period;
};

__global__ __launch_bounds__(LIN_NTH) void lin_fwd_roles(LinFwdArgs a) {
    __shared__ __attribute__((aligned(16))) unsigned char lds[LF_NS * LF_STAGE];
    const int tid = threadIdx.x, lane = tid & 63, lr = lane & 15, lk = lane >> 4;
    const int wave = __builtin_amdgcn_readfirstlane(tid >> 6);
    const int m0 = blockIdx.x * LIN_BM;
    const int ka = a.a_absmax ? pow2_scale_exp(*a.a_absmax, 12) : 0, kb = pow2_scale_exp(*a.b_absmax, 12);
    const float psa = ldexpf(1.f, ka), unscale = ldexpf(1.f, -(ka + kb));
    const int nks = a.K >> 5, nblk = a.K >> 6, kpc = a.period >> 5;
    const bool affine = a.a_scale != nullptr;
    if (wave >= 4) {
        const int st_ = tid - 256;
        const int sk = (st_ & 15) * 4;
        const bool second = sk >= 32;
        f32x4 ar[2][8];
        auto issue_a = [&](int blk, f32x4 (&r)[8]) {
#pragma unroll
            for (int i = 0; i < 8; ++i) {
                const int row = (st_ + 256 * i) >> 4;
                r[i] = (f32x4){0.f, 0.f, 0.f, 0.f};
                if (m0 + row < a.M && blk < nblk) r[i] = __builtin_nontemporal_load(reinterpret_cast<const f32x4*>(a.A + (long)(m0 + row) * a.lda + (long)blk * 64 + sk));
            }
        };
        auto commit_a = [&](int blk, const f32x4 (&r)[8]) {
            if (blk >= nblk) return;
            const int c0 = (2 * blk) / kpc, c1 = (2 * blk + 1) / kpc;
            const float sc = affine ? (second ? a.a_scale[c1] : a.a_scale[c0]) * psa : psa, sh = affine ? (second ? a.a_shift[c1] : a.a_shift[c0]) * psa : 0.f;
            const float floor_ = affine ? 0.f : -INFINITY;
            unsigned char* st = lds + (blk % LF_NS) * LF_STAGE;
#pragma unroll
            for (int i = 0; i < 8; ++i) {
                const int row = (st_ + 256 * i) >> 4;
                float x[4];
#pragma unroll
                for (int j = 0; j < 4; ++j) x[j] = __builtin_amdgcn_fmed3f(fmaxf(fmaf(r[i][j], sc, sh), floor_), -65000.f, 65000.f);
                uint2 hi, lo;
                split2_pair_f16(x[0], x[1], hi.x, lo.x);
                split2_pair_f16(x[2], x[3], hi.y, lo.y);
                *reinterpret_cast<uint2*>(st + (0 * LIN_BM + row) * LF_RS + sk * 2) = hi;
                *reinterpret_cast<uint2*>(st + (1 * LIN_BM + row) * LF_RS + sk * 2) = lo;
            }
        };
        issue_a(0, ar[0]);
        commit_a(0, ar[0]);
        issue_a(1, ar[1]); issue_a(2, ar[0]);
#pragma unroll 1
        for (int b0 = 0; b0 < nblk; b0 += 2) {
            __syncthreads();
            commit_a(b0 + 1, ar[1]); issue_a(b0 + 3, ar[1]);
            if (b0 + 1 < nblk) {
                __syncthreads();
                commit_a(b0 + 2, ar[0]); issue_a(b0 + 4, ar[0]);
            }
        }
        return;
    }
    lu32x4 bf[2][4][2];
    auto load_b = [&](int ks, lu32x4 (&dst)[4][2]) {
        if (ks >= nks) return;
#pragma unroll
        for (int nt = 0; nt < 4; ++nt)
#pragma unroll
            for (int sp = 0; sp < 2; ++sp)
                dst[nt][sp] = *reinterpret_cast<const lu32x4*>(a.planes + (((long)(wave * 4 + nt) * nks + ks) * 2 + sp) * 1024 + (unsigned)lane * 16u);
    };
    f32x4 acc[8][4];
#pragma unroll
    for (int mt = 0; mt < 8; ++mt)
#pragma unroll
        for (int nt = 0; nt < 4; ++nt) acc[mt][nt] = (f32x4){0.f, 0.f, 0.f, 0.f};
    load_b(0, bf[0]);
    auto load_af = [&](const unsigned char* st, int h, int qt, lu32x4 (&af)[2][2]) {
#pragma unroll
        for (int sp = 0; sp < 2; ++sp)
#pragma unroll
            for (int q = 0; q < 2; ++q) af[sp][q] = *reinterpret_cast<const lu32x4*>(st + (sp * LIN_BM + (qt * 2 + q) * 16 + lr) * LF_RS + h * 64 + lk * 16);
    };
    auto multiply = [&](int qt, const lu32x4 (&af)[2][2], const lu32x4 (&b)[4][2]) {
#define LR_PRODUCT(SA, SB)                                                                                                        \
        _Pragma("unroll") for (int nt = 0; nt < 4; ++nt)                                                                          \
            _Pragma("unroll") for (int q = 0; q < 2; ++q)                                                                         \
                acc[qt * 2 + q][nt] = __builtin_amdgcn_mfma_f32_16x16x32_f16(__builtin_bit_cast(f16x8, b[nt][SB]),                \
                                                                             __builtin_bit_cast(f16x8, af[SA][q]), acc[qt * 2 + q][nt], 0, 0, 0);
        LR_PRODUCT(1, 0) LR_PRODUCT(0, 1) LR_PRODUCT(0, 0)
#undef LR_PRODUCT
    };
#pragma unroll 1
    for (int blk = 0; blk < nblk; ++blk) {
        __syncthreads();
        const unsigned char* st = lds + (blk % LF_NS) * LF_STAGE;
        lu32x4 fa[2][2], fb[2][2];
        load_af(st, 0, 0, fa);
        load_b(2 * blk + 1, bf[1]);
        __builtin_amdgcn_sched_barrier(0);
        load_af(st, 0, 1, fb); multiply(0, fa, bf[0]);
        __builtin_amdgcn_sched_barrier(0);
        load_af(st, 0, 2, fa); multiply(1, fb, bf[0]);
        __builtin_amdgcn_sched_barrier(0);
        load_af(st, 0, 3, fb); multiply(2, fa, bf[0]);
        __builtin_amdgcn_sched_barrier(0);
        load_af(st, 1, 0, fa); multiply(3, fb, bf[0]);
        __builtin_amdgcn_sched_barrier(0);
        load_b(2 * blk + 2, bf[0]);
        load_af(st, 1, 1, fb); multiply(0, fa, bf[1]);
        __builtin_amdgcn_sched_barrier(0);
        load_af(st, 1, 2, fa); multiply(1, fb, bf[1]);
        __builtin_amdgcn_sched_barrier(0);
        load_af(st, 1, 3, fb); multiply(2, fa, bf[1]);
        __builtin_amdgcn_sched_barrier(0);
        multiply(3, fb, bf[1]);
        __builtin_amdgcn_sched_barrier(0);
    }
#pragma unroll
    for (int mt = 0; mt < 8; ++mt) {
        const int m = m0 + mt * 16 + lr;
        if (m >= a.M) continue;
#pragma unroll
        for (int nt = 0; nt < 4; ++nt) {
            f32x4 v = acc[mt][nt];
#pragma unroll
            for (int r = 0; r < 4; ++r) v[r] *= unscale;
            *reinterpret_cast<f32x4*>(a.C + (long)m * a.ldc + wave * 64 + nt * 16 + lk * 4) = v;
        }
    }
}

bool a2s_linear_fwd_ok(int M, int N, int K, long lda, long ldc, int period, const void* A, const void* W, const void* C) {
    return N == 256 && M >= 1 && K >= 128 && K % 64 == 0 && (period == 0 || (period % 32 == 0 && K % period == 0)) && lda % 4 == 0 && ldc % 4 == 0 &&
           (((uintptr_t)A | (uintptr_t)W | (uintptr_t)C) % 16 == 0);
}

int a2s_linear_fwd_impl(hipStream_t st, int M, int N, int K, const float* A, long lda, const float* W, float* C, long ldc, const float* a_scale,
                        const float* a_shift, int period, const float* a_absmax, const float* w_absmax, float* ws, size_t ws_bytes) {
    A2S_REQUIRE(A && W && C && w_absmax && ws && ((a_scale == nullptr) == (a_shift == nullptr)), "linear_fwd: null argument");
    A2S_REQUIRE(a2s_linear_fwd_ok(M, N, K, lda, ldc, a_scale ? period : 0, A, W, C),
                "linear_fwd: needs N = 256, K %% 64 == 0, period %% 32 == 0 and 16-byte aligned rows");
    A2S_REQUIRE(((uintptr_t)ws % 16 == 0) && ws_bytes >= (size_t)N * K * 4, "linear_fwd: workspace too small (%zu bytes needed)", (size_t)N * K * 4);
    unsigned char* planes = reinterpret_cast<unsigned char*>(ws);
    hipLaunchKernelGGL(lin_pack_planes_k, dim3((unsigned)(((long)N * (K / 8) + 255) / 256)), dim3(256), 0, st, W, (long)K, N, K, w_absmax, planes);
    A2S_CHECK_LAUNCH("lin_pack_planes_k");
    LinFwdArgs a{A, lda, planes, C, ldc, a_scale, a_shift, a_absmax, w_absmax, M, K, a_scale ? period : K};
    hipLaunchKernelGGL(lin_fwd_roles, dim3((M + LIN_BM - 1) / LIN_BM), dim3(LIN_NTH), 0, st, a);
    A2S_CHECK_LAUNCH("lin_fwd");
    return A2S_OK;
}

struct LinWgradArgs {
    const float* A; long lda;
    const unsigned char* planes;
    float* partial;
    const float* a_scale; const float* a_shift;
    const float* a_absmax; const float* d_absmax;
    int M, K, period, nblk, blk_per_split;
    long plane_stride; int np;
    float* bias_partial;
};

__global__ __launch_bounds__(256) void lin_pack_dz_planes(const float* __restrict__ dz, long ld, int M, int nsteps, const float* __restrict__ absmax,
                                                          unsigned char* __restrict__ out) {
    const long id = (long)blockIdx.x * 256 + threadIdx.x;
    const int n = (int)(id & 255), lk = (int)((id >> 8) & 3), s = (int)(id >> 10);
    if (s >= nsteps) return;
    dz += blockIdx.y * 256;
    out += (size_t)blockIdx.y * nsteps * (16 * 2 * 1024);
    float ps = ldexpf(1.f, pow2_scale_exp(*absmax, 12));
    if ((s >> 3) & 1) ps = -ps;
    float x[8];
#pragma unroll
    for (int j = 0; j < 8; ++j) {
        const int m = s * 32 + lk * 8 + j;
        x[j] = m < M ? __builtin_amdgcn_fmed3f(dz[(long)m * ld + n] * ps, -65000.f, 65000.f) : 0.f;
    }
    lu32x4 hi, lo;
#pragma unroll
    for (int i = 0; i < 4; ++i) { unsigned h, l; split2_pair_f16(x[2 * i], x[2 * i + 1], h, l); hi[i] = h; lo[i] = l; }
    unsigned char* o = out + ((((long)s * 16 + (n >> 4)) * 2) * 64 + (lk * 16 + (n & 15))) * 16;
    *reinterpret_cast<lu32x4*>(o) = hi;
    *reinterpret_cast<lu32x4*>(o + 64 * 16) = lo;
}

template <bool BIAS>
__global__ __launch_bounds__(LIN_NTH) void lin_wgrad_roles(LinWgradArgs a) {
    __shared__ __attribute__((aligned(16))) unsigned char lds[LF_NS * LF_STAGE];
    const int tid = threadIdx.x, lane = tid & 63, lr = lane & 15, lk = lane >> 4;
    const int wave = __builtin_amdgcn_readfirstlane(tid >> 6);
    const int k0 = blockIdx.x * LIN_BM;
    const int b_lo = blockIdx.y * a.blk_per_split, b_hi = min(a.nblk, b_lo + a.blk_per_split);
    const int ka = a.a_absmax ? pow2_scale_exp(*a.a_absmax, 12) : 0, kd = pow2_scale_exp(*a.d_absmax, 12);
    const float psa = ldexpf(1.f, ka), unscale = ldexpf(1.f, -(ka + kd));
    const bool affine = a.a_scale != nullptr;
    if (wave >= 4) {
        const int st_ = tid - 256;
        const int rq = st_ & 15, cq0 = st_ >> 4;
        float sc[2], sh[2];
#pragma unroll
        for (int u = 0; u < 2; ++u) {
            const int ch = affine ? (k0 + 4 * (cq0 + 16 * u)) / a.period : 0;
            sc[u] = affine ? a.a_scale[ch] * psa : psa; sh[u] = affine ? a.a_shift[ch] * psa : 0.f;
        }
        const float floor_ = affine ? 0.f : -INFINITY;
        f32x4 ar[2][8];
        f32x4 bs[2] = {(f32x4){0.f, 0.f, 0.f, 0.f}, (f32x4){0.f, 0.f, 0.f, 0.f}};
        auto issue_a = [&](int blk, f32x4 (&r)[8]) {
#pragma unroll
            for (int u = 0; u < 2; ++u)
#pragma unroll
                for (int j = 0; j < 4; ++j) {
                    const int m = blk * 64 + 4 * rq + j;
                    r[4 * u + j] = (f32x4){0.f, 0.f, 0.f, 0.f};
                    if (m < a.M && blk < b_hi) r[4 * u + j] = __builtin_nontemporal_load(reinterpret_cast<const f32x4*>(a.A + (long)m * a.lda + k0 + 4 * (cq0 + 16 * u)));
                }
        };
        auto commit_a = [&](int blk, const f32x4 (&r)[8]) {
            if (blk >= b_hi) return;
            unsigned char* st = lds + (blk % LF_NS) * LF_STAGE;
            if (BIAS) {
#pragma unroll
                for (int u = 0; u < 2; ++u)
#pragma unroll
                    for (int j = 0; j < 4; ++j)
#pragma unroll
                        for (int c = 0; c < 4; ++c) bs[u][c] += r[4 * u + j][c];
            }
#pragma unroll
            for (int u = 0; u < 2; ++u)
// ... 161 lines not shown
}
size_t a2s_linear_wgrad_ws_bytes_impl(int M, int K) {
    if (M < 1 || K < LIN_BM || K % LIN_BM) return 0;
    const size_t nsteps = 2 * (size_t)((M + 63) / 64);
    return nsteps * 16 * 2 * 1024 + (size_t)lin_wgrad_splits(M, K) * 256 * K * sizeof(float);
}
bool a2s_linear_wgrad_ok(int M, int N, int K, long ldz, long lda, long ldg, int period, const void* dz, const void* A, const void* G) {
    return N == 256 && M >= 64 && K >= LIN_BM && K % LIN_BM == 0 && (period == 0 || (period % 4 == 0 && K % period == 0)) && lda % 4 == 0 && ldg % 4 == 0 && ldz >= 256 &&
           (((uintptr_t)dz | (uintptr_t)A | (uintptr_t)G) % 16 == 0);
}
int a2s_linear_wgrad_impl(hipStream_t st, int M, int N, int K, const float* dz, long ldz, const float* A, long lda, float* G, long ldg, const float* a_scale,
                          const float* a_shift, int period, const float* dz_absmax, const float* a_absmax, float* ws, size_t ws_bytes) {
    A2S_REQUIRE(dz && A && G && dz_absmax && ws && ((a_scale == nullptr) == (a_shift == nullptr)), "linear_wgrad: null argument");
    A2S_REQUIRE(a2s_linear_wgrad_ok(M, N, K, ldz, lda, ldg, a_scale ? period : 0, dz, A, G), "linear_wgrad: needs N = 256, K %% 128 == 0, period %% 4 == 0, 16-byte aligned rows");
    A2S_REQUIRE(((uintptr_t)ws % 16 == 0) && ws_bytes >= a2s_linear_wgrad_ws_bytes_impl(M, K), "linear_wgrad: workspace too small (%zu bytes needed)",
                a2s_linear_wgrad_ws_bytes_impl(M, K));
    const int nblk = (M + 63) / 64, nsteps = 2 * nblk, splits = lin_wgrad_splits(M, K);
    unsigned char* planes = reinterpret_cast<unsigned char*>(ws);
    float* partial = reinterpret_cast<float*>(planes + (size_t)nsteps * 16 * 2 * 1024);
    hipLaunchKernelGGL(lin_pack_dz_planes, dim3((unsigned)(((long)nsteps * 1024 + 255) / 256)), dim3(256), 0, st, dz, ldz, M, nsteps, dz_absmax, planes);
    A2S_CHECK_LAUNCH("lin_pack_dz_planes");
    LinWgradArgs a{A, lda, planes, partial, a_scale, a_shift, a_absmax, dz_absmax, M, K, a_scale ? period : K, nblk, (nblk + splits - 1) / splits, 0, 256, nullptr};
    hipLaunchKernelGGL(lin_wgrad_roles<false>, dim3(K / LIN_BM, splits), dim3(LIN_NTH), 0, st, a);
    A2S_CHECK_LAUNCH("lin_wgrad");
    const long n = 256L * K;
    hipLaunchKernelGGL(lin_wgrad_reduce<false>, dim3((unsigned)((n / 4 + 255) / 256)), dim3(256), 0, st, partial, splits, n, G, ldg, K, nullptr, nullptr);
    A2S_CHECK_LAUNCH("lin_wgrad_reduce");
    return A2S_OK;
}

#define TALLK_SLAB_BYTES (64u << 20)
int a2s_tallk_wgrad_on = 1;
int a2s_tallk_wgrad_max_splits = 0;
static long long g_tallk_launches = 0;
long a2s_tallk_wgrad_launches(void) { return (long)__atomic_load_n(&g_tallk_launches, __ATOMIC_RELAXED); }

static int tallk_splits(int M, int Np, int K) {
    const int tiles = (K / LIN_BM) * (Np / 256), nblk = (M + 63) / 64;
    int cus = a2s_device_geometry().cus;
    if (cus < 1) cus = 256;
    int s = cus / tiles;
    const size_t slab = (size_t)Np * K * sizeof(float);
    if ((size_t)s * slab > TALLK_SLAB_BYTES) s = (int)(TALLK_SLAB_BYTES / slab);
    if (s > nblk) s = nblk;
    if (a2s_tallk_wgrad_max_splits > 0 && s > a2s_tallk_wgrad_max_splits) s = a2s_tallk_wgrad_max_splits;
    return s < 1 ? 1 : s;
}
bool a2s_tallk_wgrad_ok(int M, int Np, int K, long ldp, long lda, long ldg, int transposed, const void* P, const void* A, const void* G, const void* bias) {
    return a2s_tallk_wgrad_on && M >= 64 && Np >= 256 && Np % 256 == 0 && Np <= 2048 && K >= LIN_BM && K % LIN_BM == 0 && K <= 4096 && ldp >= Np && lda >= K &&
           lda % 4 == 0 && ldg % 4 == 0 && ldg >= (transposed ? Np : K) && (((uintptr_t)P | (uintptr_t)A | (uintptr_t)G | (uintptr_t)bias) % 16 == 0);
}
size_t a2s_tallk_wgrad_ws_bytes_impl(int M, int Np, int K) {
    if (M < 1 || Np < 256 || Np % 256 || K < LIN_BM || K % LIN_BM) return 0;
    const size_t nsteps = 2 * (size_t)((M + 63) / 64), splits = (size_t)tallk_splits(M, Np, K);
    return (size_t)(Np / 256) * nsteps * 16 * 2 * 1024 + splits * Np * K * sizeof(float) + splits * K * sizeof(float);
}
int a2s_tallk_wgrad_impl(hipStream_t st, int M, int Np, int K, const float* P, long ldp, const float* A, long lda, float* G, long ldg, int transposed,
                         float* bias, const float* p_absmax, const float* a_absmax, float* ws, size_t ws_bytes) {
    A2S_REQUIRE(P && A && G && p_absmax && a_absmax && ws, "tallk_wgrad: null argument");
    A2S_REQUIRE(a2s_tallk_wgrad_ok(M, Np, K, ldp, lda, ldg, transposed, P, A, G, bias),
                "tallk_wgrad: needs M >= 64, Np %% 256 == 0, K %% 128 == 0, 16-byte aligned bases and rows (or the switch \"tallk_wgrad\" is off)");
    A2S_REQUIRE(((uintptr_t)ws % 16 == 0) && ws_bytes >= a2s_tallk_wgrad_ws_bytes_impl(M, Np, K), "tallk_wgrad: workspace too small (%zu bytes needed)",
                a2s_tallk_wgrad_ws_bytes_impl(M, Np, K));
    const int nblk = (M + 63) / 64, nsteps = 2 * nblk, splits = tallk_splits(M, Np, K), npb = Np / 256;
    const size_t plane_stride = (size_t)nsteps * 16 * 2 * 1024;
    unsigned char* planes = reinterpret_cast<unsigned char*>(ws);
    float* partial = reinterpret_cast<float*>(planes + npb * plane_stride);
    float* bias_partial = partial + (size_t)splits * Np * K;
    hipLaunchKernelGGL(lin_pack_dz_planes, dim3((unsigned)(((long)nsteps * 1024 + 255) / 256), npb), dim3(256), 0, st, P, ldp, M, nsteps, p_absmax, planes);
    A2S_CHECK_LAUNCH("lin_pack_dz_planes");
    LinWgradArgs a{A, lda, planes, partial, nullptr, nullptr, a_absmax, p_absmax, M, K, K, nblk, (nblk + splits - 1) / splits, (long)plane_stride, Np,
                   bias ? bias_partial : nullptr};
    if (bias) hipLaunchKernelGGL(lin_wgrad_roles<true>, dim3(K / LIN_BM, splits, npb), dim3(LIN_NTH), 0, st, a);
    else hipLaunchKernelGGL(lin_wgrad_roles<false>, dim3(K / LIN_BM, splits, npb), dim3(LIN_NTH), 0, st, a);
    A2S_CHECK_LAUNCH("lin_wgrad (tall-K)");
    const long n = (long)Np * K, nthreads = (n + (bias ? K : 0)) / 4;
    const dim3 rgrid((unsigned)((nthreads + 255) / 256));
    if (transposed) hipLaunchKernelGGL(lin_wgrad_reduce<true>, rgrid, dim3(256), 0, st, partial, splits, n, G, ldg, K, bias ? bias_partial : nullptr, bias);
    else hipLaunchKernelGGL(lin_wgrad_reduce<false>, rgrid, dim3(256), 0, st, partial, splits, n, G, ldg, K, bias ? bias_partial : nullptr, bias);
    A2S_CHECK_LAUNCH("lin_wgrad_reduce");
    __atomic_fetch_add(&g_tallk_launches, 1LL, __ATOMIC_RELAXED);
    return A2S_OK;
}
```

### piano_a2s_amd/engine.py

```python
import ctypes as C
import random as _py_random
import threading

import torch

from . import hip
from .spec import EOS, PAD, SOS, VOCAB_SIZE


def plan_note_steps(gt_rows, max_steps):
    B = gt_rows.shape[0]
    is_eos = gt_rows == EOS
    first = torch.where(is_eos.any(1), is_eos.float().argmax(1), torch.full((B,), max_steps))
    steps = int(first.max()) + 1 if bool((first < max_steps).all()) else max_steps
    steps = min(steps, max_steps)
    idx = torch.arange(1, steps + 1, dtype=torch.long)
    last = (is_eos[:, :steps].long() * idx).amax(dim=1)
    lengths = torch.where(last > 0, last, torch.full((B,), max_steps, dtype=torch.long))
    return steps, lengths


import os as _os

_GREEDY_GRAPH = _os.environ.get("A2S_GREEDY_GRAPH") == "1"
# ... 246 lines not shown
    @staticmethod
    def check_counts(count, dev):
        import torch.distributed as dist
        t = torch.tensor([float(count), -float(count)], dtype=torch.float64, device=dev)
        dist.all_reduce(t, op=dist.ReduceOp.MAX)
        hi, lo = float(t[0]), -float(t[1])
        if hi != lo:
            raise RuntimeError(f"synchronised BatchNorm: the ranks hold different numbers of frames in this step ({lo:.0f} .. {hi:.0f}); "
                               "give every rank the same batch shape (DistributedSampler pads; drop or pad an uneven last batch)")

    @staticmethod
    def _empty(*shape, dev, dtype=torch.float32):
        return torch.empty(shape, dtype=dtype, device=dev)

    def _bn(self, S, name, partial, nblocks, C_, count, training):
        dev = S[name + ".weight"].device
        mean, invstd, scale, shift = (self._empty(C_, dev=dev) for _ in range(4))
        L = hip.lib()
        self.bn_counts = getattr(self, "bn_counts", {})
        if training and self.sync_bn:
            partial, count = self._global_stats(partial, nblocks, C_, count)
            nblocks = 1
        self.bn_counts[name] = count
        hip.check(L.a2s_bn_finalize(hip.stream(), hip._p(partial), nblocks, C_, count, hip._p(S[name + ".weight"]), hip._p(S[name + ".bias"]),
                                    hip._p(S[name + ".running_mean"]), hip._p(S[name + ".running_var"]), hip._p(S[name + ".num_batches_tracked"]), hip._p(mean),
                                    hip._p(invstd), hip._p(scale), hip._p(shift), 1e-5, 0.1, 1 if training else 0), "a2s_bn_finalize")
        return mean, invstd, scale, shift

    def convstack(self, S, spec_in, training, drop_mask=None):
        L = hip.lib()
        B, _, T, F = spec_in.shape
        dev = spec_in.device
        x = spec_in.contiguous()
        chans = [(1, 20), (20, 20), (20, 40), (40, 40)]
        scale = shift = None
        saved = {"x0": x, "y": [], "bn": [], "yabs": []}
        yabs = None
        for i, (ci, co) in enumerate(chans, start=1):
            y = self._empty(B, T, co, F, dev=dev)
            nblk = L.a2s_conv3x3_stat_blocks(B, T, F, ci)
            partial = self._empty(nblk, co, 2, dev=dev) if training else None
            cws = hip.conv_workspace(ci, dev)
            yabs_out = self._empty(co, dev=dev)
            hip.conv3x3_forward(x.view(B, T, ci, F), S[f"convstack.conv{i}.weight"], y, scale, shift, partial, cws, yabs, yabs_out)
            mean, invstd, scale, shift = self._bn(S, f"convstack.bn{i}", partial, nblk, co, float(B) * T * F, training)
            saved["y"].append(y)
            saved["bn"].append((mean, invstd, scale, shift))
            saved["yabs"].append(yabs_out)
            saved.setdefault("abound", []).append(hip.act_bound(scale, shift, yabs_out))
            x, yabs = y, yabs_out
        y4 = x.view(B * T, 40 * F)
        Cf = self.cfg["conv_feature_size"]
        a4 = None
        saved["w_out_amax"] = hip.absmax(S["convstack.out.weight"])
        z = hip.linear_forward(y4, S["convstack.out.weight"], (scale, shift, F), saved["abound"][3], saved["w_out_amax"])
        rows = B * T
        rpb = 64
        nblk = (rows + rpb - 1) // rpb
        partial = None
        if training:
            partial = self._empty(nblk, Cf, 2, dev=dev)
            hip.check(L.a2s_col_stats(hip.stream(), hip._p(z), hip._p(partial), rows, Cf, rpb), "a2s_col_stats")
        mean, invstd, scale, shift = self._bn(S, "convstack.out_bn", partial, nblk, Cf, float(rows), training)
        out = self._empty(rows, Cf, dev=dev)
        hip.check(L.a2s_bn1d_relu_dropout(hip.stream(), hip._p(z), hip._p(out), hip._p(scale), hip._p(shift), hip._p(drop_mask), 1.0 / 0.8, out.numel(), Cf),
                  "a2s_bn1d_relu_dropout")
        saved.update(a4=a4, z=z, out_bn=(mean, invstd, scale, shift), drop=drop_mask)
        return out.view(B, T, Cf), saved

    def encoder(self, S, x, training):
        L = hip.lib()
        B, T, _ = x.shape
        H = self.cfg["hidden_size"]
        dev = x.device
        saved = {"layers": []}
        gws = [hip.gemm_workspace(B, dev), hip.gemm_workspace(B, dev)]
        streams = encoder_streams(dev, B)
        inp = x.reshape(B * T, -1)
        finals = []
        for layer in (0, 1):
            out = self._empty(B, T, 2 * H, dev=dev)
            lsave = {"in": inp, "dirs": []}
            in_amax = (hip.absmax(inp) if layer == 0 else hip.one(dev)) if _ENC_TWO_TERM else None
            gis = [hip.linear(inp, S[f"encoder.gru.weight_ih_{sfx}"], S[f"encoder.gru.bias_ih_{sfx}"],
                              two_term=(in_amax, hip.absmax(S[f"encoder.gru.weight_ih_{sfx}"])) if _ENC_TWO_TERM else None)
                   for sfx in (f"l{layer}", f"l{layer}_reverse")]
            def direction(d, sfx, gi):
                hbuf = self._empty(2, B, H, dev=dev)
                gh = self._empty(B, 3 * H, dev=dev)
                hn = self._empty(B, H, dev=dev)
                gates = self._empty(T, B, 4 * H, dev=dev) if training else None
                hip.check(L.a2s_gru_seq_fwd(hip.stream(), hip._p(gi), T * 3 * H, 3 * H, hip._p(S[f"encoder.gru.weight_hh_{sfx}"]),
                                            hip._p(S[f"encoder.gru.bias_hh_{sfx}"]), C.c_void_p(out.data_ptr() + 4 * d * H), T * 2 * H, 2 * H, hip._p(hbuf), hip._p(gh),
                                            hip._p(gates), hip._p(hn), B, T, H, d, hip._p(gws[d]), gws[d].numel() * 4), "a2s_gru_seq_fwd")
                return {"gi": gi, "gates": gates, "hn": hn, "scratch": (hbuf, gh)}

            join = fork_on_streams(dev, streams, [lambda d=d, sfx=sfx: direction(d, sfx, gis[d])
                                                  for d, sfx in enumerate((f"l{layer}", f"l{layer}_reverse"))])
            for rec in join():
                finals.append(rec["hn"])
                lsave["dirs"].append(rec)
            lsave["out"] = out
            saved["layers"].append(lsave)
            inp = out.view(B * T, 2 * H)
        W, bias = S["encoder.fc.weight"], S["encoder.fc.bias"]
        hidden = self._empty(B, 2 * H, dev=dev)
        for l in (0, 1):
            hf, hr = finals[2 * l], finals[2 * l + 1]
            hip.gemm(hf, H, 1, W, 1, 2 * H, hidden, 2 * H, B, H, H, bias=bias, c_off=l * H)
            hip.gemm(hr, H, 1, W, 1, 2 * H, hidden, 2 * H, B, H, H, beta=1.0, act=2, b_off=H, c_off=l * H)
        saved["finals"] = finals
        saved["hidden"] = hidden
        return saved["layers"][1]["out"], hidden, saved

    def _keys(self, S, prefix, enc2d, H):
        W = S[prefix + ".attn.weight"]
        K = self._empty(enc2d.shape[0], H, dev=enc2d.device)
        hip.gemm(enc2d, 2 * H, 1, W, 1, 4 * H, K, H, enc2d.shape[0], H, 2 * H, b_off=2 * H, act=3,
                 two_term=(hip.one(enc2d.device), hip.absmax(W)) if _ENC_TWO_TERM else None)
        return K

    def _staff_token(self, S, ids, lengths, len_stride, out, col0, maxlen, id_bstride, ids_are_i64, record=None):
        L = hip.lib()
        names = [f"decoder.staff_emb.{w}_{sfx}" for sfx in ("l0", "l0_reverse") for w in ("weight_ih", "weight_hh", "bias_ih", "bias_hh")]
        arr = (C.c_void_p * 8)(*[S[n].data_ptr() for n in names])
        R = out.shape[0]
        E, Sz = self.cfg["note_emb_size"], self.cfg["staff_emb_size"]
        hsave = torch.empty((R, 2, maxlen, Sz), dtype=torch.float32, device=out.device) if record is not None else None
        hip.check(L.a2s_staff_emb_fwd(hip.stream(), hip._p(S["decoder.note_emb.weight"]), arr, hip._p(ids) if ids_are_i64 else None,
                                      None if ids_are_i64 else hip._p(ids), id_bstride, hip._p(lengths), len_stride, hip._p(out), out.stride(0), col0, hip._p(hsave), R,
                                      maxlen, E, Sz), "a2s_staff_emb_fwd")
        if record is not None:
            record.append(dict(ids=ids, lengths=lengths, len_stride=len_stride, col0=col0, maxlen=maxlen, id_bstride=id_bstride,
                               i64=ids_are_i64, hsave=hsave))

    def _decode_staff(self, S, prefix, keys, enc, h0, max_steps, probs_bar, gt_bar, steps, tf_flags, training, drop_p, B, T, attn_ws=None, gemm_ws=None,
                      active=None, drop=None, flags_dev=None, persist=False, defer_launch=False):
        L = hip.lib()
        H, E, V = self.cfg["hidden_size"], self.cfg["note_emb_size"], VOCAB_SIZE
        H2, ldx = 2 * H, E + 2 * H
        dev = enc.device
        n = steps
        graph = gt_bar is None and not training and getattr(self, "greedy_graph", _GREEDY_GRAPH)
        grammar = self.kern_grammar if (gt_bar is None and not training) else None
        if grammar is not None:
            if grammar.vocab_size != V:
                raise hip.A2SError(f"Engine.kern_grammar is a table over {grammar.vocab_size} symbols, the decoder's vocabulary has {V}")
            persist = False
        align = bool(self.alignment) and not training
        if align:
            if active is not None or defer_launch:
                raise hip.A2SError("alignment decodes bar by bar: no fused bars, no pair loop")
            persist, graph = False, False
        if gt_bar is None and not training and self._beam_slots():
            if active is not None or defer_launch:
                raise hip.A2SError("beam search decodes bar by bar: no fused bars, no pair loop")
            ids_, lengths_, saved = self._decode_staff_beam(S, prefix, keys, enc, h0, max_steps, probs_bar, n, B, T, grammar, self._beam_slots())
            if align:
                gt_ids = ids_.long()
                n_forced = plan_note_steps(gt_ids.cpu(), max_steps)[0]
                scratch = torch.zeros((B, max_steps, V), dtype=torch.float32, device=dev)
                forced = self._decode_staff(S, prefix, keys, enc, h0, max_steps, scratch, gt_ids, n_forced, [1] * n_forced, False, 0.0, B, T,
                                            attn_ws=attn_ws, gemm_ws=gemm_ws)[2]
                saved["align"], saved["align_forced"] = forced["align"], forced
            return ids_, lengths_, saved
        t_base = torch.zeros(1, dtype=torch.int32, device=dev) if graph else None
# ... 515 lines not shown
```

### piano_a2s_amd/engine_bwd.py

```python
import ctypes as C
import os
import threading

import torch

from . import hip
from .spec import SOS, VOCAB_SIZE


def _os_env(name, default):
    return os.environ.get(name, default)


def _ptr(t, off=0):
    return C.c_void_p(t.data_ptr() + 4 * off)


_COLSUM_WS = {}


def _colsum(x, ld, out, rows, ncol, x_off=0, out_off=0, beta=1.0):
    ws = None
    if rows >= 2048:
        key = (x.device, torch.cuda.current_stream().cuda_stream, threading.get_ident())
# ... 437 lines not shown
                        assert not bool(gf[:late_join].any()), f"clip group {gi}: non-decoder gradients in the group buffer would be lost by the late fold"
        defer = True
        d_conv = _encoder_bwd(eng, S, G, sv["enc"], dEnc, d_hid_carry, B, T, wait_weight_grads=not defer)
        n_conv = next(off for k, off in zip(names, offs) if not k.startswith("convstack."))
        if grad_ready is not None:
            if defer:
                with torch.cuda.stream(_weight_grad_stream(dev)):
                    grad_ready(self.flat_full, n_conv, total + 1)
            else:
                grad_ready(self.flat_full, n_conv, total + 1)
        if getattr(eng, "conv_unperm", None) is not None:
            d_conv = d_conv.reshape(B, T, -1).index_select(0, eng.conv_unperm)
        _convstack_bwd(eng, S, G, sv["conv"], d_conv, B, T, F)
        if defer:
            torch.cuda.current_stream().wait_stream(_weight_grad_stream(dev))
        if grad_ready is not None:
            grad_ready(flat, 0, n_conv)
        G[None] = flat
        G["__loss_gate__"] = self.flat_full[total:]
        eng._keep_alive = self.keep_alive
        return G




def backward(eng, S, grad_outputs, grad_ready=None, loss_total=None):
    from .engine import group_views, run_clip_groups
    sv = eng.saved
    assert sv["training"], "backward needs a forward run with training=True (batch statistics / saved activations)"
    dev = sv["enc_out"].device
    clip_groups = sv.get("clip_groups") or [(0, sv["shape"][0])]
    ctx = Backward(eng, S, sv["shape"], dev, clip_groups, sv.get("concurrent"), sv.get("bar_major"))
    dts, dkey, dup, dlo = [g.contiguous() for g in grad_outputs]

    def group(gidx):
        b0, b1 = clip_groups[gidx]
        if ctx.bar_major:
            dup_g, dlo_g = group_views(dup, clip_groups, gidx), group_views(dlo, clip_groups, gidx)
        else:
            dup_g, dlo_g = dup[b0:b1], dlo[b0:b1]
        ctx.decoder_group(gidx, sv["groups"][gidx], dts[b0:b1], dkey[b0:b1], dup_g, dlo_g)

    run_clip_groups(dev, [lambda gi=gi: group(gi) for gi in range(len(clip_groups))])
    if loss_total is not None:
        ctx.flat_full[ctx.total:].copy_(loss_total.reshape(1))
    return ctx.finish(grad_ready)


_WG_STREAMS = {}
_DEFERRED_STREAMS = {}


def _deferred_streams(dev, group=0):
    idx = torch.device(dev).index if torch.device(dev).index is not None else torch.cuda.current_device()
    key = (idx, group)
    if key not in _DEFERRED_STREAMS:
        _DEFERRED_STREAMS[key] = (torch.cuda.Stream(device=idx), torch.cuda.Stream(device=idx))
    return _DEFERRED_STREAMS[key]



def _weight_grad_stream(dev):
    from .engine import group_stream
    return group_stream(dev, 1)


def _encoder_bwd(eng, S, G, es, dEnc, d_hidden, B, T, wait_weight_grads=True):
    L = hip.lib()
    H = eng.cfg["hidden_size"]
    dev = dEnc.device
    W = S["encoder.fc.weight"]
    dpre = torch.empty_like(d_hidden)
    hip.check(L.a2s_ew_act_bwd(hip.stream(), hip._p(d_hidden), hip._p(es["hidden"]), hip._p(dpre), dpre.numel(), 2), "tanh bwd")
    dhn = []
    for l in (0, 1):
        for half, hfin in enumerate((es["finals"][2 * l], es["finals"][2 * l + 1])):
            d = torch.empty((B, H), device=dev)
            hip.gemm(dpre, 2 * H, 1, W, 2 * H, 1, d, H, B, H, H, a_off=l * H, b_off=half * H)
            hip.gemm(dpre, 1, 2 * H, hfin, H, 1, G["encoder.fc.weight"], 2 * H, H, H, B, beta=1.0, a_off=l * H, c_off=half * H)
            dhn.append(d)
        _colsum(dpre, 2 * H, G["encoder.fc.bias"], B, H, x_off=l * H)
    gws = [hip.gemm_workspace(B, dev), hip.gemm_workspace(B, dev)]
    two_term = True
    in_amax = hip.absmax(es["layers"][0]["in"]) if two_term else None
    dout = dEnc
    for layer in (1, 0):
        ls = es["layers"][layer]
        inp = ls["in"]
        I = inp.shape[1]
        out = ls["out"]
        dX = torch.empty((B * T, I), device=dev)
        from .engine import encoder_streams, fork_on_streams
        streams = encoder_streams(dev, B)

        def direction(d, sfx):
            dgi = torch.empty((B, T, 3 * H), device=dev)
            dghs = torch.empty((B, T, 3 * H), device=dev)
            dgh_first, dhbuf, dgh_tmp = torch.empty((B, 3 * H), device=dev), torch.empty((2, B, H), device=dev), torch.empty((B, 3 * H), device=dev)
            ranges, valid = torch.empty(2, device=dev), C.c_int(0)
            if two_term and L.a2s_debug_get(b"tallk_wgrad") > 0:
                hip.check(L.a2s_gru_seq_bwd_ranged(hip.stream(), _ptr(dout, d * H), T * 2 * H, 2 * H, _ptr(out, d * H), T * 2 * H, 2 * H, hip._p(ls["dirs"][d]["gates"]),
                                                   hip._p(S[f"encoder.gru.weight_hh_{sfx}"]), hip._p(dhn[2 * layer + d]), hip._p(dgi), hip._p(dghs), hip._p(dgh_first),
                                                   hip._p(dhbuf), hip._p(dgh_tmp), B, T, H, d, hip._p(gws[d]), gws[d].numel() * 4, hip._p(ranges), C.byref(valid)),
                          "a2s_gru_seq_bwd_ranged")
            else:
                hip.check(L.a2s_gru_seq_bwd(hip.stream(), _ptr(dout, d * H), T * 2 * H, 2 * H, _ptr(out, d * H), T * 2 * H, 2 * H, hip._p(ls["dirs"][d]["gates"]),
                                            hip._p(S[f"encoder.gru.weight_hh_{sfx}"]), hip._p(dhn[2 * layer + d]), hip._p(dgi), hip._p(dghs), hip._p(dgh_first),
                                            hip._p(dhbuf), hip._p(dgh_tmp), B, T, H, d, hip._p(gws[d]), gws[d].numel() * 4), "a2s_gru_seq_bwd")
            return (dgi, dghs, dgh_first, dhbuf, dgh_tmp, ranges if valid.value else None)

        res = fork_on_streams(dev, streams, [lambda d=d, sfx=sfx: direction(d, sfx) for d, sfx in enumerate((f"l{layer}", f"l{layer}_reverse"))])()
        dgi_amax = []
        for d, sfx in enumerate((f"l{layer}", f"l{layer}_reverse")):
            dgi2 = res[d][0].view(B * T, 3 * H)
            Wih = S[f"encoder.gru.weight_ih_{sfx}"]
            ranges = res[d][5]
            tt = (ranges[0:1] if ranges is not None else hip.absmax(dgi2), hip.absmax(Wih)) if two_term else None
            dgi_amax.append(tt[0] if tt else None)
            if L.a2s_debug_get(b"gemm_bf16x3") > 0:
                hip.gemm(dgi2, 3 * H, 1, Wih.t().contiguous(), 1, 3 * H, dX, I, B * T, I, 3 * H, beta=0.0 if d == 0 else 1.0, two_term=tt)
            else:
                hip.gemm(dgi2, 3 * H, 1, Wih, I, 1, dX, I, B * T, I, 3 * H, beta=0.0 if d == 0 else 1.0, two_term=tt)
        wg = _weight_grad_stream(dev)
        ev = torch.cuda.Event()
        ev.record()
        wg.wait_event(ev)
        for d, sfx in enumerate((f"l{layer}", f"l{layer}_reverse")):
            dgi, dghs, dgh_first, ranges = res[d][0], res[d][1], res[d][2], res[d][5]
            for t in (dgi, dghs, dgh_first, dgi_amax[d], in_amax, ranges):
                if t is not None:
                    t.record_stream(wg)
            with torch.cuda.stream(wg):
                dgi2, dghs2 = dgi.view(B * T, 3 * H), dghs.view(B * T, 3 * H)
                x_bound = ((in_amax if layer == 0 else hip.one(dev)) if two_term else None)
                if not hip.tallk_wgrad(inp, 0, I, dgi2, 0, 3 * H, G[f"encoder.gru.weight_ih_{sfx}"], 0, I, B * T, I, 3 * H, x_bound, dgi_amax[d],
                                       transposed=True, bias=G[f"encoder.gru.bias_ih_{sfx}"]):
                    _linear_bwd(inp, S[f"encoder.gru.weight_ih_{sfx}"], dgi2, G, f"encoder.gru.weight_ih_{sfx}", f"encoder.gru.bias_ih_{sfx}",
                                dy_amax=dgi_amax[d], x_bound=x_bound)
                dghs_amax = (ranges[1:2] if ranges is not None else hip.absmax(dghs2)) if two_term else None
                if not hip.tallk_wgrad(out, d * H, 2 * H, dghs2, 0, 3 * H, G[f"encoder.gru.weight_hh_{sfx}"], 0, H, B * T, H, 3 * H,
                                       hip.one(dev) if two_term else None, dghs_amax, transposed=True, bias=G[f"encoder.gru.bias_hh_{sfx}"]):
                    sk = L.a2s_gemm_pick_splitk(3 * H, H, B * T, 1)
                    hip.gemm(dghs2, 1, 3 * H, out, 2 * H, 1, G[f"encoder.gru.weight_hh_{sfx}"], H, 3 * H, H, B * T, beta=1.0, splitk=sk, b_off=d * H,
                             two_term=(dghs_amax, hip.one(dev)) if two_term else None)
                    _colsum(dghs2, 3 * H, G[f"encoder.gru.bias_hh_{sfx}"], B * T, 3 * H)
                _colsum(dgh_first, 3 * H, G[f"encoder.gru.bias_hh_{sfx}"], B, 3 * H)
        dout = dX.view(B, T, I)
    if wait_weight_grads:
        torch.cuda.current_stream().wait_stream(_weight_grad_stream(dev))
    return dout


_FUSE_BN_APPLY = False
_FUSE_BN_APPLY_L1 = True
_DGRAD_BNSTATS = True
_SYNC_FUSED = True
_LIN_WGRAD_AT = "before"
_FUSE_BN_ROWS = os.environ.get("A2S_FUSE_BN_ROWS", "1") != "0"


def _linear_dgrad_generic(L, dev, rows, F, Cf, dz, Wout, da, y4, bn4, dz_amax, w_amax):
    nblk = L.a2s_gemm_bnstats_blocks(rows, F)
    part = torch.empty((nblk, 40, 2), dtype=torch.float32, device=dev)
    if L.a2s_debug_get(b"gemm_bf16x3") > 0:
        Wt = Wout.t().contiguous()
        wb, s_bk, s_bn = Wt, 1, Cf
    else:
# ... 158 lines not shown
```

### piano_a2s_amd/hip.py

```python
import ctypes as C
import os
import threading

import torch

from .abi import PROTOTYPES, STRUCTS, A2SError
from .build import LIB

LIB = os.environ.get("A2S_LIB", LIB)

NoteDecArgs, NoteDecBwdArgs, BeamArgs, AlignArgs = (STRUCTS[n] for n in ("a2s_note_dec_args", "a2s_note_dec_bwd_args", "a2s_beam_args", "a2s_align_args"))
_lib = None


def lib():
    global _lib
    if _lib is None:
        if not os.path.exists(LIB):
            raise A2SError(f"HIP extension not built: {LIB} is missing (run `python __graft_entry__.py build`). "
                           "There is no CPU fallback for the transcription hot path.")
        arith = os.environ.get("A2S_ARITH", "f16x2")
        if arith not in ("f16x2", "bf16x3", "f32"):
            raise A2SError(f"A2S_ARITH={arith!r}: expected f16x2, bf16x3 or f32")
        L = C.CDLL(LIB)
# ... 441 lines not shown
    _need(1 <= C <= 8, fn, "channels", f"must be in 1 .. 8 (got {C})")
    _need(1 <= L <= 4096, fn, "table", f"must have 1 .. 4096 rows (got {L})")
    _need(1 <= K <= 8192, fn, "table", f"must have 1 .. 8192 columns (got {K})")
    _need(1 <= M <= 4096, fn, "M", f"must be in 1 .. 4096 (got {M})")
    _need(0 <= Hh < K, fn, "Hh", f"must be in 0 .. K - 1 = {K - 1} (got {Hh})")
    _need(torch.is_tensor(n_in) and n_in.dtype == torch.int32 and n_in.dim() == 1 and n_in.is_contiguous() and n_in.device == table.device, fn, "n_in",
          "must be a contiguous int32 tensor of one element per clip on the table's device")
    B = n_in.shape[0]
    _need(torch.is_tensor(x) and x.dim() == 2, fn, "x", "must be a 2-D float32 tensor of interleaved frames")
    nim = x.shape[1] // C if n_in_max is None else int(n_in_max)
    _need(nim >= 0, fn, "n_in_max", f"must be >= 0 (got {nim})")
    nom = -(-nim * L // M) if n_out_max is None else int(n_out_max)
    _need(nom >= 1 or B == 0, fn, "n_out_max", f"must be >= 1 (got {nom})")
    xs = _rows(fn, "x", x, B, nim * C, table.device)
    if y is None:
        y = torch.empty((B, max(nom, 0)), dtype=torch.float32, device=table.device)
    ys = _rows(fn, "y", y, B, nom, table.device)
    if B == 0:
        return y
    _need(x.data_ptr() != y.data_ptr(), fn, "y", "must not be x (the resampler works out of place)")
    check(lib().a2s_resample_rows(stream(), _p(x), xs, _p(n_in), nim, C, _p(table), L, M, K, Hh, _p(y), ys, nom, B), "a2s_resample_rows")
    return y


def resample_tile_samples():
    return int(lib().a2s_resample_tile_samples())


def resample_launches():
    return int(lib().a2s_resample_launches())


def note_match(ref, ref_off, hyp, hyp_off, n_pairs, dur_ticks, midi, cls, out):
    fn = "note_match"
    for name, t, dtype in (("ref", ref, torch.int32), ("hyp", hyp, torch.int32), ("ref_off", ref_off, torch.int64), ("hyp_off", hyp_off, torch.int64)):
        _need(isinstance(t, int) or (torch.is_tensor(t) and t.dtype == dtype and t.is_contiguous()), fn, name, f"must be a contiguous {dtype} tensor or an address")
    for name, t in (("ref_off", ref_off), ("hyp_off", hyp_off)):
        _need(isinstance(t, int) or t.numel() == n_pairs + 1, fn, name, f"must have n_pairs + 1 = {n_pairs + 1} elements")
    for name, t in (("dur_ticks", dur_ticks), ("midi", midi), ("cls", cls)):
        _need(torch.is_tensor(t) and t.dtype == torch.int32 and t.is_contiguous() and t.dim() == 1 and t.numel() == dur_ticks.numel(), fn, name,
              "must be a contiguous int32 tensor (V,)")
    _need(torch.is_tensor(out) and out.dtype == torch.int32 and out.is_contiguous() and out.numel() == 8 * n_pairs, fn, "out",
          f"must be a contiguous int32 tensor of 8 * n_pairs = {8 * n_pairs} elements")
    if n_pairs == 0:
        return out
    check(lib().a2s_note_match(stream(), _p(ref), _p(ref_off), _p(hyp), _p(hyp_off), n_pairs, _p(dur_ticks), _p(midi), _p(cls), dur_ticks.numel(), _p(out)),
          "a2s_note_match")
    return out


def note_match_launches():
    return int(lib().a2s_note_match_launches())


def align_buffers(R, max_steps, T, device):
    t = dict(attw_step=torch.zeros((R, T), dtype=torch.float32, device=device),
             peak=torch.full((R, max_steps), -1, dtype=torch.int32, device=device),
             weight=torch.zeros((R, max_steps), dtype=torch.float32, device=device),
             centroid=torch.full((R, max_steps), -1.0, dtype=torch.float32, device=device))
    g = AlignArgs()
    for name in ("attw_step", "peak", "weight", "centroid"):
        setattr(g, name, t[name].data_ptr())
    g.out_stride = max_steps
    g.next_state, g.n_states, g.row_state = None, 0, None
    return g, t


def check(rc, what):
    if rc != 0:
        raise A2SError(f"{what} failed ({rc}): {lib().a2s_last_error().decode()}")


def f32(x):
    return C.c_float(float(x))


def gemm(A, sAm, sAk, B, sBk, sBn, Cout, ldc, M, N, K, alpha=1.0, beta=0.0, bias=None, act=0,
         batch=1, bsA=0, bsB=0, bsC=0, splitk=1, a_off=0, b_off=0, c_off=0, a_affine=None, b_affine=None, two_term=None):
    L = lib()
    ws, ws_bytes = None, 0
    if splitk > 1:
        ws_bytes = L.a2s_gemm_workspace_bytes(M, N, batch, splitk)
        ws = torch.empty(ws_bytes // 4, dtype=torch.float32, device=Cout.device)
    pa = C.c_void_p(A.data_ptr() + 4 * a_off)
    pb = C.c_void_p(B.data_ptr() + 4 * b_off)
    pc = C.c_void_p(Cout.data_ptr() + 4 * c_off)
    if a_affine is None and b_affine is None and two_term is None:
        check(L.a2s_gemm_f32(stream(), M, N, K, alpha, pa, sAm, sAk, pb, sBk, sBn, beta, pc, ldc, _p(bias), act, batch, bsA, bsB, bsC, splitk, _p(ws), ws_bytes),
              "a2s_gemm_f32")
        return
    asc, ash, ap = a_affine if a_affine is not None else (None, None, 0)
    bsc, bsh, bp = b_affine if b_affine is not None else (None, None, 0)
    if two_term is not None:
        check(L.a2s_gemm_f32_affine_scaled(stream(), M, N, K, alpha, pa, sAm, sAk, pb, sBk, sBn, beta, pc, ldc, _p(bias), act, batch, bsA, bsB, bsC, splitk, _p(ws),
                                           ws_bytes, _p(asc), _p(ash), ap, _p(bsc), _p(bsh), bp, _p(two_term[0]), _p(two_term[1])), "a2s_gemm_f32_affine_scaled")
        return
    check(L.a2s_gemm_f32_affine(stream(), M, N, K, alpha, pa, sAm, sAk, pb, sBk, sBn, beta, pc, ldc, _p(bias), act, batch, bsA, bsB, bsC, splitk, _p(ws), ws_bytes,
                                _p(asc), _p(ash), ap, _p(bsc), _p(bsh), bp), "a2s_gemm_f32_affine")


_ONES = {}


def one(device):
    key = torch.device(device).index
    if key not in _ONES:
        _ONES[key] = torch.ones(1, dtype=torch.float32, device=device)
    return _ONES[key]


def absmax(x, out=None):
    if out is None:
        out = torch.empty(1, dtype=torch.float32, device=x.device)
    check(lib().a2s_absmax(stream(), _p(x), x.numel(), _p(out)), "a2s_absmax")
    return out


def linear(x2d, weight, bias=None, act=0, out=None, beta=0.0, x_affine=None, two_term=None):
    M, K = x2d.shape
    N = weight.shape[0]
    if out is None:
        out = torch.empty((M, N), dtype=torch.float32, device=x2d.device)
    gemm(x2d, x2d.stride(0), x2d.stride(1), weight, weight.stride(1), weight.stride(0), out, out.stride(0), M, N, K,
         bias=bias, act=act, beta=beta, a_affine=x_affine, two_term=two_term)
    return out


def conv3x3_forward(x, w, y, scale, shift, partial, cws, in_absmax=None, out_absmax=None):
    B, T, Cin, F = x.shape
    check(lib().a2s_conv3x3_ranged(stream(), _p(x), _p(w), _p(y), _p(scale), _p(shift), _p(in_absmax), _p(partial), _p(out_absmax),
                                   B, T, F, Cin, y.shape[2], _p(cws)), "a2s_conv3x3_ranged")


def conv3x3_dgrad_for_test(dy, w, yl):
    L = lib()
    B, T, Cout, F = dy.shape
    Cin = w.shape[1]
    dev = dy.device
    dx = torch.full((B, T, Cin, F), float("nan"), device=dev)
    amax = absmax(dy)
    part = torch.zeros(L.a2s_conv3x3_stat_blocks(B, T, F, Cout), Cin, 2, device=dev)
    cws = conv_workspace(Cout, dev)
    zeros, ones = torch.zeros(Cin, device=dev), torch.ones(Cin, device=dev)
    check(L.a2s_conv3x3_dgrad_bnstats_scaled(stream(), _p(dy), _p(w), _p(dx), _p(yl), _p(zeros), _p(ones), _p(ones), _p(zeros), _p(part),
                                             B, T, F, Cout, Cin, _p(cws), _p(amax)), "a2s_conv3x3_dgrad_bnstats_scaled")
    torch.cuda.synchronize()
    return dx


def act_bound(scale, shift, x_absmax):
    out = torch.empty(1, dtype=torch.float32, device=scale.device)
    check(lib().a2s_act_bound(stream(), _p(scale), _p(shift), _p(x_absmax), scale.numel(), _p(out)), "a2s_act_bound")
    return out


def conv3x3_wgrad(dy, x, scale, shift, dW, ws, dy_absmax, act_absmax):
    B, T, Cout, F = dy.shape
    Cin = x.shape[2]
    check(lib().a2s_conv3x3_wgrad_ranged(stream(), _p(dy), _p(x), _p(scale), _p(shift), _p(dW), _p(ws), ws.numel() * 4, B, T, F, Cin, Cout, _p(dy_absmax),
                                         _p(act_absmax)), "a2s_conv3x3_wgrad_ranged")


def conv3x3_wgrad_for_test(dy, x, scale, shift):
    L = lib()
    B, T, Cout, F = dy.shape
    Cin = x.shape[2]
# ... 66 lines not shown
```

Before: 637.7.

## Add LDS-resident two-term f16 GEMM path for encoder input projections

Routes unscaled two-term encoder GEMMs (K of 256 or 512, or K a multiple of 256 with N a multiple of 256) to new kernels. These pack the weight into f16 hi/lo planes once and keep the whole A row-block resident in LDS while sweeping all N tiles. A generalized variant of the linear-forward roles kernel with a fused bias/activation epilogue is also added. The backward pass reuses the saved input absmax instead of recomputing it. The aim is to cut repeated A loads and the generic big-tile GEMM overhead, at the cost of a per-call weight-packing launch and a workspace allocation.

```diff
diff --git a/include/a2s.h b/include/a2s.h
--- a/include/a2s.h
+++ b/include/a2s.h
@@ -51,6 +51,7 @@
 int a2s_absmax(void* stream, const float* x, long n, float* out);
 int a2s_gemm_bnstats_blocks(int M, int period);
 size_t a2s_gemm_workspace_bytes(int M, int N, int batch, int splitk);
+size_t a2s_gemm_resident_ws_bytes(int M, int N, int K, long sAm, long sAk, long sBk, long sBn, long ldc, int batch, int splitk);
 int a2s_gemm_pick_splitk(int M, int N, int K, int batch);
 void a2s_gemm_debug_tile(int cfg);
 int a2s_debug_set(const char* key, int value);
diff --git a/piano_a2s_amd/csrc/a2s_api.hip b/piano_a2s_amd/csrc/a2s_api.hip
--- a/piano_a2s_amd/csrc/a2s_api.hip
+++ b/piano_a2s_amd/csrc/a2s_api.hip
@@ -78,6 +78,9 @@
 }
 int a2s_gemm_bnstats_blocks(int M, int period) { return a2s_cdiv(M, 128) * a2s_gemm_bnstats_slots(period); }
 size_t a2s_gemm_workspace_bytes(int M, int N, int batch, int splitk) { return a2s_gemm_workspace_bytes_impl(M, N, batch, splitk); }
+size_t a2s_gemm_resident_ws_bytes(int M, int N, int K, long sAm, long sAk, long sBk, long sBn, long ldc, int batch, int splitk) {
+    return a2s_gemm_resident_ws_bytes_impl(M, N, K, sAm, sAk, sBk, sBn, ldc, batch, splitk);
+}
 int a2s_gemm_pick_splitk(int M, int N, int K, int batch) { return a2s_gemm_pick_splitk_impl(M, N, K, batch); }
 void a2s_gemm_debug_tile(int cfg) { a2s_gemm_debug_tile_impl(cfg); }
 size_t a2s_note_step_workspace_floats(int H, int E) { return a2s_note_step_workspace_floats_impl(H, E); }
@@ -87,6 +90,7 @@
     if (id >= 0) { a2s_switch_store(id, value); return A2S_OK; }
     if (!strcmp(key, "attn_deferred_fast")) { a2s_attn_deferred_fast = value ? 1 : 0; return A2S_OK; }
     if (!strcmp(key, "tallk_wgrad")) { a2s_tallk_wgrad_on = value ? 1 : 0; return A2S_OK; }
+    if (!strcmp(key, "enc_resident")) { a2s_enc_resident_on = (value >= 0 && value <= 3) ? value : 1; return A2S_OK; }
     if (!strcmp(key, "tallk_wgrad_max_splits")) { a2s_tallk_wgrad_max_splits = value > 0 ? value : 0; return A2S_OK; }
     if (!strcmp(key, "gemm_tile")) { a2s_gemm_debug_tile_impl(value); return A2S_OK; }
     snprintf(a2s_err_msg, sizeof(a2s_err_msg), "a2s_debug_set: unknown key %s", key);
@@ -108,6 +112,8 @@
     if (!strcmp(key, "attn_pair_bwd_launches")) return (int)a2s_attn_pair_bwd_launches();
     if (!strcmp(key, "attn_deferred_fast")) return a2s_attn_deferred_fast;
     if (!strcmp(key, "tallk_wgrad")) return a2s_tallk_wgrad_on;
+    if (!strcmp(key, "enc_resident")) return a2s_enc_resident_on;
+    if (!strcmp(key, "enc_resident_launches")) return (int)a2s_enc_resident_launches();
     if (!strcmp(key, "tallk_wgrad_max_splits")) return a2s_tallk_wgrad_max_splits;
     if (!strcmp(key, "tallk_wgrad_launches")) return (int)a2s_tallk_wgrad_launches();
     if (!strcmp(key, "attn_dk_ahead_launches")) return (int)a2s_attn_dk_ahead_launches();
diff --git a/piano_a2s_amd/csrc/a2s_common.h b/piano_a2s_amd/csrc/a2s_common.h
--- a/piano_a2s_amd/csrc/a2s_common.h
+++ b/piano_a2s_amd/csrc/a2s_common.h
@@ -170,6 +170,14 @@
     return fmaf(-2.f, __builtin_amdgcn_rcpf(e + 1.f), 1.f);
 }
 __device__ __forceinline__ float exp2x_clamped(float x) { return __expf(2.f * fminf(fmaxf(x, -43.f), 43.f)); }
+__device__ __forceinline__ float gemm_epilogue_value(float acc, float alpha, float bias, float beta, float old, int act) {
+    float x = alpha * acc + bias;
+    if (beta != 0.f) x += beta * old;
+    if (act == 1) x = fmaxf(x, 0.f);
+    else if (act == 2) x = fast_tanh(x);
+    else if (act == 3) x = exp2x_clamped(x);
+    return x;
+}
 __device__ __forceinline__ float tanh_ek(float ek, float eq) { return fmaf(-2.f, __builtin_amdgcn_rcpf(fmaf(ek, eq, 1.f)), 1.f); }
 __device__ __forceinline__ float sech2_ek(float ek, float eq) {
     const float r = __builtin_amdgcn_rcpf(fmaf(ek, eq, 1.f));
diff --git a/piano_a2s_amd/csrc/a2s_gemm.hip b/piano_a2s_amd/csrc/a2s_gemm.hip
--- a/piano_a2s_amd/csrc/a2s_gemm.hip
+++ b/piano_a2s_amd/csrc/a2s_gemm.hip
@@ -415,14 +415,8 @@
                     }
                 }
 #pragma unroll
-                for (int r = 0; r < 4; ++r) {
-                    float x = g.alpha * v[r] + ((g.bias && n + r < g.N) ? g.bias[n + r] : 0.f);
-                    if (g.beta != 0.f) x += g.beta * old[r];
-                    if (g.act == 1) x = fmaxf(x, 0.f);
-                    else if (g.act == 2) x = fast_tanh(x);
-                    else if (g.act == 3) x = exp2x_clamped(x);
-                    v[r] = x;
-                }
+                for (int r = 0; r < 4; ++r)
+                    v[r] = gemm_epilogue_value(v[r], g.alpha, (g.bias && n + r < g.N) ? g.bias[n + r] : 0.f, g.beta, old[r], g.act);
             }
             if (full) *reinterpret_cast<f32x4*>(dst) = v;
             else {
@@ -546,6 +540,17 @@
     return splitk > 1 ? (size_t)batch * splitk * M * N * sizeof(float) : 0;
 }
 
+static int g_force_tile = 0;
+void a2s_gemm_debug_tile_impl(int cfg) { g_force_tile = cfg; }
+
+size_t a2s_gemm_resident_ws_bytes_impl(int M, int N, int K, long sAm, long sAk, long sBk, long sBn, long ldc, int batch, int splitk) {
+    if (M <= 0 || N <= 0 || K <= 0 || g_force_tile) return 0;
+    GemmArgs g = {};
+    g.M = M; g.N = N; g.K = K; g.batch = batch; g.splitk = splitk; g.two_term = 1; g.vecA = g.vecB = 1;
+    if (!big_two_term_ok(g, true, true)) return 0;
+    return a2s_enc_resident_ok(M, N, K, sAm, sAk, sBk, sBn, ldc, batch, splitk, nullptr, nullptr, nullptr) ? a2s_enc_resident_ws_bytes_impl(N, K) : 0;
+}
+
 int a2s_gemm_pick_splitk_impl(int M, int N, int K, int batch) {
     const long tiles = (long)a2s_cdiv(M, 64) * a2s_cdiv(N, 64) * batch;
     if (K < 4096) return 1;
@@ -578,9 +583,6 @@
 
 int a2s_gemm_bnstats_slots(int period) { return period > 0 ? (period + 127) / 128 + 1 : 0; }
 
-static int g_force_tile = 0;
-void a2s_gemm_debug_tile_impl(int cfg) { g_force_tile = cfg; }
-
 int a2s_gemm_affine_impl(hipStream_t st, int M, int N, int K, float alpha, const float* A, long sAm, long sAk,
                   const float* B, long sBk, long sBn, float beta, float* C, long ldc, const float* bias, int act,
                   int batch, long bsA, long bsB, long bsC, int splitk, float* ws, size_t ws_bytes,
@@ -590,6 +592,7 @@
     if (M <= 0 || N <= 0 || batch <= 0) return A2S_OK;
     A2S_REQUIRE(K >= 0 && A && B && C, "gemm: null operand or negative K");
     A2S_REQUIRE(splitk >= 0, "gemm: splitk must be >= 0 (0 = choose automatically when a workspace is given)");
+    const int splitk_asked = splitk;
     const bool mid = M > 64 && M <= 2048 && batch == 1 && N <= 2048;
     int mid_tile = 0;
     if (mid) mid_tile = M <= 1024 ? 2 : 3;
@@ -644,7 +647,12 @@
     g.vecA = (akc ? (sAk == 1 && aligned(A, sAm, bsA)) : (sAm == 1 && aligned(A, sAk, bsA))) ? 1 : 0;
     g.vecB = (bkc ? (sBk == 1 && aligned(B, sBn, bsB)) : (sBn == 1 && aligned(B, sBk, bsB))) ? 1 : 0;
 
-    if (!g_force_tile && big_two_term_ok(g, akc, bkc)) launch_big_two_term(g, akc, bkc, st);
+    if (!g_force_tile && big_two_term_ok(g, akc, bkc)) {
+        if (splitk_asked == 1 && !a_scale && !b_scale && !ep_y && ws && b_absmax && ((uintptr_t)ws % 16 == 0) && ws_bytes >= a2s_enc_resident_ws_bytes_impl(N, K) &&
+            a2s_enc_resident_ok(M, N, K, sAm, sAk, sBk, sBn, ldc, batch, splitk_asked, A, B, C))
+            return a2s_enc_resident_impl(st, M, N, K, alpha, A, sAm, B, sBn, beta, C, ldc, bias, act, a_absmax, b_absmax, ws, ws_bytes);
+        launch_big_two_term(g, akc, bkc, st);
+    }
     else if (ep_y) launch_cfg<128, 128, 2, 2>(g, akc, bkc, st);
     else if (!g_force_tile && mid_tile == 2 && g.splitk >= 1 && M * (long)N < (1L << 22)) launch_cfg<64, 32, 4, 1>(g, akc, bkc, st);
     else if (!g_force_tile && mid_tile == 3 && M * (long)N < (1L << 22)) launch_cfg<64, 64, 2, 2>(g, akc, bkc, st);
diff --git a/piano_a2s_amd/csrc/a2s_internal.h b/piano_a2s_amd/csrc/a2s_internal.h
--- a/piano_a2s_amd/csrc/a2s_internal.h
+++ b/piano_a2s_amd/csrc/a2s_internal.h
@@ -22,6 +22,7 @@
     const float* a_scale, const float* a_shift, int a_period, const float* b_scale, const float* b_shift, int b_period,
     const float* ep_y, const float* ep_mean, const float* ep_invstd, const float* ep_scale, const float* ep_shift,
     float* ep_partial, int ep_period, int two_term, const float* a_absmax, const float* b_absmax);
+size_t a2s_gemm_resident_ws_bytes_impl(int M, int N, int K, long sAm, long sAk, long sBk, long sBn, long ldc, int batch, int splitk);
 int a2s_gemm_impl(hipStream_t st, int M, int N, int K, float alpha, const float* A, long sAm, long sAk,
     const float* B, long sBk, long sBn, float beta, float* C, long ldc, const float* bias, int act,
     int batch, long bsA, long bsB, long bsC, int splitk, float* ws, size_t ws_bytes);
@@ -46,6 +47,12 @@
 bool a2s_tallk_wgrad_ok(int M, int Np, int K, long ldp, long lda, long ldg, int transposed, const void* P, const void* A, const void* G, const void* bias);
 int a2s_tallk_wgrad_impl(hipStream_t st, int M, int Np, int K, const float* P, long ldp, const float* A, long lda, float* G, long ldg, int transposed,
     float* bias, const float* p_absmax, const float* a_absmax, float* ws, size_t ws_bytes);
+extern int a2s_enc_resident_on;
+long a2s_enc_resident_launches(void);
+size_t a2s_enc_resident_ws_bytes_impl(int N, int K);
+bool a2s_enc_resident_ok(int M, int N, int K, long sAm, long sAk, long sBk, long sBn, long ldc, int batch, int splitk, const void* A, const void* B, const void* C);
+int a2s_enc_resident_impl(hipStream_t st, int M, int N, int K, float alpha, const float* A, long lda, const float* B, long ldb, float beta, float* C, long ldc,
+    const float* bias, int act, const float* a_absmax, const float* b_absmax, float* ws, size_t ws_bytes);
 
 int a2s_act_bound_impl(hipStream_t st, const float* scale, const float* shift, const float* absmax, int C, float* out);
 size_t a2s_conv3x3_workspace_floats_impl(int Cin);
diff --git a/piano_a2s_amd/csrc/a2s_linear.hip b/piano_a2s_amd/csrc/a2s_linear.hip
--- a/piano_a2s_amd/csrc/a2s_linear.hip
+++ b/piano_a2s_amd/csrc/a2s_linear.hip
@@ -26,7 +26,7 @@
     const int kgroups = K >> 3, nks = K >> 5;
     const int n = (int)(id / kgroups), kg = (int)(id % kgroups);
     if (n >= N) return;
-    const float ps = ldexpf(1.f, pow2_scale_exp(*absmax, 12));
+    const float ps = ldexpf(1.f, absmax ? pow2_scale_exp(*absmax, 12) : 0);
     const f32x4 v0 = *reinterpret_cast<const f32x4*>(W + (long)n * ld + kg * 8);
     const f32x4 v1 = *reinterpret_cast<const f32x4*>(W + (long)n * ld + kg * 8 + 4);
     float x[8];
@@ -214,13 +214,17 @@
     const float* a_scale; const float* a_shift;
     const float* a_absmax; const float* b_absmax;
     int M, K, period;
+    const float* bias; float alpha, beta; int act, ncb;
 };
 
+template <bool GEN>
 __global__ __launch_bounds__(LIN_NTH) void lin_fwd_roles(LinFwdArgs a) {
     __shared__ __attribute__((aligned(16))) unsigned char lds[LF_NS * LF_STAGE];
     const int tid = threadIdx.x, lane = tid & 63, lr = lane & 15, lk = lane >> 4;
     const int wave = __builtin_amdgcn_readfirstlane(tid >> 6);
-    const int m0 = blockIdx.x * LIN_BM;
+    const int nb = GEN ? (int)(blockIdx.x >> 3) % a.ncb : 0;
+    const int m0 = (GEN ? (int)((blockIdx.x >> 3) / a.ncb) * 8 + (int)(blockIdx.x & 7) : (int)blockIdx.x) * LIN_BM;
+    if (GEN && m0 >= a.M) return;
     const int ka = a.a_absmax ? pow2_scale_exp(*a.a_absmax, 12) : 0, kb = pow2_scale_exp(*a.b_absmax, 12);
     const float psa = ldexpf(1.f, ka), unscale = ldexpf(1.f, -(ka + kb));
     const int nks = a.K >> 5, nblk = a.K >> 6, kpc = a.period >> 5;
@@ -244,12 +248,15 @@
             const float sc = affine ? (second ? a.a_scale[c1] : a.a_scale[c0]) * psa : psa, sh = affine ? (second ? a.a_shift[c1] : a.a_shift[c0]) * psa : 0.f;
             const float floor_ = affine ? 0.f : -INFINITY;
             unsigned char* st = lds + (blk % LF_NS) * LF_STAGE;
+            const float ps = ((blk >> 2) & 1) ? -psa : psa;
 #pragma unroll
             for (int i = 0; i < 8; ++i) {
                 const int row = (st_ + 256 * i) >> 4;
                 float x[4];
 #pragma unroll
-                for (int j = 0; j < 4; ++j) x[j] = __builtin_amdgcn_fmed3f(fmaxf(fmaf(r[i][j], sc, sh), floor_), -65000.f, 65000.f);
+                for (int j = 0; j < 4; ++j)
+                    x[j] = GEN ? __builtin_amdgcn_fmed3f(r[i][j] * ps, -65000.f, 65000.f)
+                               : __builtin_amdgcn_fmed3f(fmaxf(fmaf(r[i][j], sc, sh), floor_), -65000.f, 65000.f);
                 uint2 hi, lo;
                 split2_pair_f16(x[0], x[1], hi.x, lo.x);
                 split2_pair_f16(x[2], x[3], hi.y, lo.y);
@@ -278,13 +285,22 @@
         for (int nt = 0; nt < 4; ++nt)
 #pragma unroll
             for (int sp = 0; sp < 2; ++sp)
-                dst[nt][sp] = *reinterpret_cast<const lu32x4*>(a.planes + (((long)(wave * 4 + nt) * nks + ks) * 2 + sp) * 1024 + (unsigned)lane * 16u);
+                dst[nt][sp] = *reinterpret_cast<const lu32x4*>(a.planes + (((long)(nb * 16 + wave * 4 + nt) * nks + ks) * 2 + sp) * 1024 + (unsigned)lane * 16u);
     };
     f32x4 acc[8][4];
 #pragma unroll
     for (int mt = 0; mt < 8; ++mt)
 #pragma unroll
         for (int nt = 0; nt < 4; ++nt) acc[mt][nt] = (f32x4){0.f, 0.f, 0.f, 0.f};
+    bool neg = false;
+    auto flip = [&]() {
+#pragma unroll
+        for (int mt = 0; mt < 8; ++mt)
+#pragma unroll
+            for (int nt = 0; nt < 4; ++nt)
+#pragma unroll
+                for (int r = 0; r < 4; ++r) acc[mt][nt][r] = -acc[mt][nt][r];
+    };
     load_b(0, bf[0]);
     auto load_af = [&](const unsigned char* st, int h, int qt, lu32x4 (&af)[2][2]) {
 #pragma unroll
@@ -303,6 +319,10 @@
     };
 #pragma unroll 1
     for (int blk = 0; blk < nblk; ++blk) {
+        if (GEN) {
+            const bool want = (blk >> 2) & 1;
+            if (want != neg) { flip(); neg = want; }
+        }
         __syncthreads();
         const unsigned char* st = lds + (blk % LF_NS) * LF_STAGE;
         lu32x4 fa[2][2], fb[2][2];
@@ -326,6 +346,32 @@
         __builtin_amdgcn_sched_barrier(0);
         multiply(3, fb, bf[1]);
         __builtin_amdgcn_sched_barrier(0);
+    }
+    if (GEN) {
+        if (neg) flip();
+        float bv[4][4];
+#pragma unroll
+        for (int nt = 0; nt < 4; ++nt)
+#pragma unroll
+            for (int r = 0; r < 4; ++r) bv[nt][r] = a.bias ? a.bias[nb * 256 + wave * 64 + nt * 16 + lk * 4 + r] : 0.f;
+#pragma unroll
+        for (int mt = 0; mt < 8; ++mt) {
+            const int m = m0 + mt * 16 + lr;
+            if (m >= a.M) continue;
+#pragma unroll
+            for (int nt = 0; nt < 4; ++nt) {
+                float* dst = a.C + (long)m * a.ldc + nb * 256 + wave * 64 + nt * 16 + lk * 4;
+                f32x4 v = acc[mt][nt];
+#pragma unroll
+                for (int r = 0; r < 4; ++r) v[r] *= unscale;
+                f32x4 old = {0.f, 0.f, 0.f, 0.f};
+                if (a.beta != 0.f) old = *reinterpret_cast<const f32x4*>(dst);
+#pragma unroll
+                for (int r = 0; r < 4; ++r) v[r] = gemm_epilogue_value(v[r], a.alpha, bv[nt][r], a.beta, old[r], a.act);
+                *reinterpret_cast<f32x4*>(dst) = v;
+            }
+        }
+        return;
     }
 #pragma unroll
     for (int mt = 0; mt < 8; ++mt) {
@@ -355,8 +401,8 @@
     unsigned char* planes = reinterpret_cast<unsigned char*>(ws);
     hipLaunchKernelGGL(lin_pack_planes_k, dim3((unsigned)(((long)N * (K / 8) + 255) / 256)), dim3(256), 0, st, W, (long)K, N, K, w_absmax, planes);
     A2S_CHECK_LAUNCH("lin_pack_planes_k");
-    LinFwdArgs a{A, lda, planes, C, ldc, a_scale, a_shift, a_absmax, w_absmax, M, K, a_scale ? period : K};
-    hipLaunchKernelGGL(lin_fwd_roles, dim3((M + LIN_BM - 1) / LIN_BM), dim3(LIN_NTH), 0, st, a);
+    LinFwdArgs a{A, lda, planes, C, ldc, a_scale, a_shift, a_absmax, w_absmax, M, K, a_scale ? period : K, nullptr, 1.f, 0.f, 0, 1};
+    hipLaunchKernelGGL(lin_fwd_roles<false>, dim3((M + LIN_BM - 1) / LIN_BM), dim3(LIN_NTH), 0, st, a);
     A2S_CHECK_LAUNCH("lin_fwd");
     return A2S_OK;
 }
@@ -684,3 +730,167 @@
     __atomic_fetch_add(&g_tallk_launches, 1LL, __ATOMIC_RELAXED);
     return A2S_OK;
 }
+
+int a2s_enc_resident_on = 1;
+static long long g_enc_resident_launches = 0;
+long a2s_enc_resident_launches(void) { return (long)__atomic_load_n(&g_enc_resident_launches, __ATOMIC_RELAXED); }
+
+struct EncResArgs {
+    const float* A; long lda;
+    const unsigned char* planes;
+    float* C; long ldc;
+    const float* bias;
+    const float* a_absmax; const float* b_absmax;
+    int M, N, act;
+    float alpha, beta;
+};
+
+template <int KK, int BM>
+__global__ __launch_bounds__(LIN_NTH) void enc_resident(EncResArgs a) {
+    constexpr int NKS = KK / 32, NBLK = KK / 128, MT = BM / 16, KQ = KK / 4;
+    static_assert(NBLK * 2 * BM * LIN_RS == LIN_LDS && BM * KQ == 16 * LIN_NTH && MT % 4 == 0, "enc_resident: BM rows x KK fill the LDS image and 16 float4 per thread");
+    __shared__ __attribute__((aligned(16))) unsigned char lds[LIN_LDS];
+    const int tid = threadIdx.x, lane = tid & 63, wave = tid >> 6, lr = lane & 15, lk = lane >> 4;
+    const int m0 = blockIdx.x * BM;
+    const int ka = a.a_absmax ? pow2_scale_exp(*a.a_absmax, 12) : 0, kb = a.b_absmax ? pow2_scale_exp(*a.b_absmax, 12) : 0;
+    const float psa = ldexpf(1.f, ka), unscale = ldexpf(1.f, -(ka + kb));
+
+    {
+        f32x4 v[16];
+#pragma unroll
+        for (int i = 0; i < 16; ++i) {
+            const int slot = tid + LIN_NTH * i, row = slot / KQ, k = (slot % KQ) * 4;
+            v[i] = (f32x4){0.f, 0.f, 0.f, 0.f};
+            if (m0 + row < a.M) v[i] = *reinterpret_cast<const f32x4*>(a.A + (long)(m0 + row) * a.lda + k);
+        }
+#pragma unroll
+        for (int i = 0; i < 16; ++i) {
+            const int slot = tid + LIN_NTH * i, row = slot / KQ, k = (slot % KQ) * 4;
+            const float ps = ((k >> 8) & 1) ? -psa : psa;
+            float x[4];
+#pragma unroll
+            for (int j = 0; j < 4; ++j) x[j] = __builtin_amdgcn_fmed3f(v[i][j] * ps, -65000.f, 65000.f);
+            uint2 hi, lo;
+            split2_pair_f16(x[0], x[1], hi.x, lo.x);
+            split2_pair_f16(x[2], x[3], hi.y, lo.y);
+            const int blk = k >> 7, off = (k & 127) * 2;
+            *reinterpret_cast<uint2*>(lds + ((blk * 2 + 0) * BM + row) * LIN_RS + off) = hi;
+            *reinterpret_cast<uint2*>(lds + ((blk * 2 + 1) * BM + row) * LIN_RS + off) = lo;
+        }
+    }
+    __syncthreads();
+
+    const int ntiles = (a.N + 255) >> 8;
+    lu32x4 bf[3][2][2];
+    auto load_b = [&](int n0, int ks, lu32x4 (&dst)[2][2]) {
+        const unsigned char* bp = a.planes + (long)(n0 >> 4) * NKS * 2 * 64 * 16;
+#pragma unroll
+        for (int nt = 0; nt < 2; ++nt)
+#pragma unroll
+            for (int sp = 0; sp < 2; ++sp) dst[nt][sp] = *reinterpret_cast<const lu32x4*>(bp + ((long)(nt * NKS + ks) * 2 + sp) * 1024 + (unsigned)lane * 16u);
+    };
+    if (wave * 32 < a.N) { load_b(wave * 32, 0, bf[0]); load_b(wave * 32, 1, bf[1]); }
+    for (int j = 0; j < ntiles; ++j) {
+        const int n0 = j * 256 + wave * 32;
+        if (n0 >= a.N) break;
+        f32x4 acc[MT][2];
+#pragma unroll
+        for (int mt = 0; mt < MT; ++mt)
+#pragma unroll
+            for (int nt = 0; nt < 2; ++nt) acc[mt][nt] = (f32x4){0.f, 0.f, 0.f, 0.f};
+        auto flip = [&]() {
+#pragma unroll
+            for (int mt = 0; mt < MT; ++mt)
+#pragma unroll
+                for (int nt = 0; nt < 2; ++nt)
+#pragma unroll
+                    for (int r = 0; r < 4; ++r) acc[mt][nt][r] = -acc[mt][nt][r];
+        };
+        bool neg = false;
+#pragma unroll
+        for (int ks = 0; ks < NKS; ++ks) {
+            if (ks + 2 < NKS) load_b(n0, ks + 2, bf[(ks + 2) % 3]);
+            const bool want = (ks >> 3) & 1;
+            if (want != neg) { flip(); neg = want; }
+#pragma unroll
+            for (int half = 0; half < MT / 4; ++half) {
+                lu32x4 af[2][4];
+#pragma unroll
+                for (int sp = 0; sp < 2; ++sp)
+#pragma unroll
+                    for (int q = 0; q < 4; ++q)
+                        af[sp][q] = *reinterpret_cast<const lu32x4*>(lds + (((ks >> 2) * 2 + sp) * BM + (half * 4 + q) * 16 + lr) * LIN_RS + (ks & 3) * 64 + lk * 16);
+#define ENC_PRODUCT(SA, SB)                                                                                                   \
+                _Pragma("unroll") for (int nt = 0; nt < 2; ++nt)                                                              \
+                    _Pragma("unroll") for (int q = 0; q < 4; ++q)                                                             \
+                        acc[half * 4 + q][nt] = __builtin_amdgcn_mfma_f32_16x16x32_f16(__builtin_bit_cast(f16x8, bf[ks % 3][nt][SB]), \
+                                                                                       __builtin_bit_cast(f16x8, af[SA][q]), acc[half * 4 + q][nt], 0, 0, 0);
+                ENC_PRODUCT(1, 0) ENC_PRODUCT(0, 1) ENC_PRODUCT(0, 0)
+#undef ENC_PRODUCT
+            }
+        }
+        if (neg) flip();
+        if (n0 + 256 < a.N) { load_b(n0 + 256, 0, bf[0]); load_b(n0 + 256, 1, bf[1]); }
+        float bv[2][4];
+#pragma unroll
+        for (int nt = 0; nt < 2; ++nt)
+#pragma unroll
+            for (int r = 0; r < 4; ++r) bv[nt][r] = a.bias ? a.bias[n0 + nt * 16 + lk * 4 + r] : 0.f;
+#pragma unroll
+        for (int mt = 0; mt < MT; ++mt) {
+            const int m = m0 + mt * 16 + lr;
+            if (m >= a.M) continue;
+#pragma unroll
+            for (int nt = 0; nt < 2; ++nt) {
+                float* dst = a.C + (long)m * a.ldc + n0 + nt * 16 + lk * 4;
+                f32x4 v = acc[mt][nt];
+#pragma unroll
+                for (int r = 0; r < 4; ++r) v[r] *= unscale;
+                f32x4 old = {0.f, 0.f, 0.f, 0.f};
+                if (a.beta != 0.f) old = *reinterpret_cast<const f32x4*>(dst);
+#pragma unroll
+                for (int r = 0; r < 4; ++r) v[r] = gemm_epilogue_value(v[r], a.alpha, bv[nt][r], a.beta, old[r], a.act);
+                *reinterpret_cast<f32x4*>(dst) = v;
+            }
+        }
+    }
+}
+
+size_t a2s_enc_resident_ws_bytes_impl(int N, int K) { return (N > 0 && K > 0) ? (size_t)N * K * 2 * 2 : 0; }
+
+static int enc_kernel_choice(int N, int K) {
+    const bool res = (K == 256 || K == 512) && N >= 32 && N % 32 == 0;
+    const bool roles = K >= 256 && K % 256 == 0 && K <= 4096 && N >= 256 && N % 256 == 0 && N <= 1024;
+    if (res && roles) return a2s_enc_resident_on == 2 ? 2 : a2s_enc_resident_on == 3 ? 1 : (N == 256 ? 2 : 1);
+    return res ? 1 : roles ? 2 : 0;
+}
+
+bool a2s_enc_resident_ok(int M, int N, int K, long sAm, long sAk, long sBk, long sBn, long ldc, int batch, int splitk, const void* A, const void* B, const void* C) {
+    return a2s_enc_resident_on && M >= 1 && N >= 1 && K >= 1 && enc_kernel_choice(N, K) != 0 && sAk == 1 && sBk == 1 && batch == 1 && splitk == 1 &&
+           sAm >= K && sBn >= K && ldc >= N && sAm % 4 == 0 && sBn % 4 == 0 && ldc % 4 == 0 && (((uintptr_t)A | (uintptr_t)B | (uintptr_t)C) % 16 == 0);
+}
+
+int a2s_enc_resident_impl(hipStream_t st, int M, int N, int K, float alpha, const float* A, long lda, const float* B, long ldb, float beta, float* C, long ldc,
+                          const float* bias, int act, const float* a_absmax, const float* b_absmax, float* ws, size_t ws_bytes) {
+    A2S_REQUIRE(A && B && C && ws && b_absmax, "enc_resident: null argument");
+    A2S_REQUIRE(a2s_enc_resident_ok(M, N, K, lda, 1, 1, ldb, ldc, 1, 1, A, B, C),
+                "enc_resident: needs K = 256 / 512 and N %% 32 == 0, or K %% 256 == 0 and N %% 256 == 0; k-contiguous operands, 16-byte aligned rows (or the switch \"enc_resident\" is off)");
+    A2S_REQUIRE(((uintptr_t)ws % 16 == 0) && ws_bytes >= a2s_enc_resident_ws_bytes_impl(N, K), "enc_resident: workspace too small (%zu bytes needed)",
+                a2s_enc_resident_ws_bytes_impl(N, K));
+    unsigned char* planes = reinterpret_cast<unsigned char*>(ws);
+    hipLaunchKernelGGL(lin_pack_planes_k, dim3((unsigned)(((long)N * (K / 8) + 255) / 256)), dim3(256), 0, st, B, ldb, N, K, b_absmax, planes);
+    A2S_CHECK_LAUNCH("lin_pack_planes_k");
+    if (enc_kernel_choice(N, K) == 2) {
+        const int ncb = N / 256, groups = ((M + LIN_BM - 1) / LIN_BM + 7) / 8;
+        LinFwdArgs f{A, lda, planes, C, ldc, nullptr, nullptr, a_absmax, b_absmax, M, K, K, bias, alpha, beta, act, ncb};
+        hipLaunchKernelGGL(lin_fwd_roles<true>, dim3((unsigned)(groups * 8 * ncb)), dim3(LIN_NTH), 0, st, f);
+        A2S_CHECK_LAUNCH("lin_fwd_roles<true>");
+    } else {
+        EncResArgs a{A, lda, planes, C, ldc, bias, a_absmax, b_absmax, M, N, act, alpha, beta};
+        if (K == 256) hipLaunchKernelGGL((enc_resident<256, 128>), dim3((M + 127) / 128), dim3(LIN_NTH), 0, st, a);
+        else hipLaunchKernelGGL((enc_resident<512, 64>), dim3((M + 63) / 64), dim3(LIN_NTH), 0, st, a);
+        A2S_CHECK_LAUNCH("enc_resident");
+    }
+    __atomic_fetch_add(&g_enc_resident_launches, 1LL, __ATOMIC_RELAXED);
+    return A2S_OK;
+}
diff --git a/piano_a2s_amd/engine.py b/piano_a2s_amd/engine.py
--- a/piano_a2s_amd/engine.py
+++ b/piano_a2s_amd/engine.py
@@ -352,6 +352,7 @@
             out = self._empty(B, T, 2 * H, dev=dev)
             lsave = {"in": inp, "dirs": []}
             in_amax = (hip.absmax(inp) if layer == 0 else hip.one(dev)) if _ENC_TWO_TERM else None
+            lsave["in_amax"] = in_amax
             gis = [hip.linear(inp, S[f"encoder.gru.weight_ih_{sfx}"], S[f"encoder.gru.bias_ih_{sfx}"],
                               two_term=(in_amax, hip.absmax(S[f"encoder.gru.weight_ih_{sfx}"])) if _ENC_TWO_TERM else None)
                    for sfx in (f"l{layer}", f"l{layer}_reverse")]
diff --git a/piano_a2s_amd/engine_bwd.py b/piano_a2s_amd/engine_bwd.py
--- a/piano_a2s_amd/engine_bwd.py
+++ b/piano_a2s_amd/engine_bwd.py
@@ -543,7 +543,9 @@
         _colsum(dpre, 2 * H, G["encoder.fc.bias"], B, H, x_off=l * H)
     gws = [hip.gemm_workspace(B, dev), hip.gemm_workspace(B, dev)]
     two_term = True
-    in_amax = hip.absmax(es["layers"][0]["in"]) if two_term else None
+    in_amax = es["layers"][0].get("in_amax")
+    if in_amax is None and two_term:
+        in_amax = hip.absmax(es["layers"][0]["in"])
     dout = dEnc
     for layer in (1, 0):
         ls = es["layers"][layer]
diff --git a/piano_a2s_amd/hip.py b/piano_a2s_amd/hip.py
--- a/piano_a2s_amd/hip.py
+++ b/piano_a2s_amd/hip.py
@@ -547,6 +547,10 @@
     if splitk > 1:
         ws_bytes = L.a2s_gemm_workspace_bytes(M, N, batch, splitk)
         ws = torch.empty(ws_bytes // 4, dtype=torch.float32, device=Cout.device)
+    elif two_term is not None and a_affine is None and b_affine is None:
+        ws_bytes = L.a2s_gemm_resident_ws_bytes(M, N, K, sAm, sAk, sBk, sBn, ldc, batch, splitk)
+        if ws_bytes:
+            ws = torch.empty(ws_bytes // 4, dtype=torch.float32, device=Cout.device)
     pa = C.c_void_p(A.data_ptr() + 4 * a_off)
     pb = C.c_void_p(B.data_ptr() + 4 * b_off)
     pc = C.c_void_p(Cout.data_ptr() + 4 * c_off)
```

Result: no change. 640.6 (median of 6 runs) (+0.5%).
